# kekeliu-whu/Wildcat-SLAM

Measured on AMD Instinct MI355X. Metric: surfel-extract Mpts/s, higher is better.
Workload: dtype f64; 1 GPU; C2: 1M-pt single scan (G2 patch lattice, 999936 pts -> 31248 surfels) per GPU, voxel-grid + 3-level octree + per-cell 3x3 PCA; input = the reference's 48-byte hilti_ros::Point records, consumed in place; points_per_gpu=999936, surfels_per_gpu=31248, parallelism=sweep-per-gpu x1

## Files before the change

### wildcat-slam_amd/csrc/ctx.h

```cpp
#pragma once
#include <hip/hip_runtime.h>

#include <cstdarg>
#include <cstdio>
#include <cstdlib>
#include <cstring>
#include <string>
#include <vector>

#include "../../include/wildcat_hip.h"
#include "extract_plan.h"

struct wc_window_state;

struct wc_buf {
  void *p = nullptr;
  size_t cap = 0;
  bool pooled = false;
  bool plain = false;
};

#ifdef WC_DEV_KNOBS
#define WC_DBG(P, bit) ((P).dbg & (bit))
#else
#define WC_DBG(P, bit) 0
#endif

struct wc_dev_opts {
  int exact_sums = 0;
  int debug_skip = 0;
  int fx_merge_min = 3;
  int fx_split = -1;
  int no_bucket_sort = 0;
  int ex_sync = 0;
  int match_pair_serial = 0;
  int lm_dense = 0;
  int lm_side_stream = 1;
  int lm_one_collective = 0;
  int map_mom_pts = 1;
  int map_lin_groups = 0;
  int map_score_groups = 0;
  int map_cast_groups = 0;
  int map_carve_groups = 0;
  int map_remove_groups = 0;
  int map_absorb_groups = 0;
  int lm_dense_radius = 7;
  int lm_radius0 = -1;
};
inline bool wc_log_env(const char *name) { return getenv(name) != nullptr; }

struct wc_ctx {
  int device = 0;
  wc_params P;
  wc_dev_opts dev;
  bool pool_ok = false;
  hipMemPool_t pool = nullptr;
  hipStream_t own_stream = nullptr;
  hipStream_t stream = nullptr;
  hipEvent_t ev0 = nullptr, ev1 = nullptr;
  std::string err;
  wc_buf b_ex_ctrl;
  wc_buf b_keys[2], b_vals[2], b_sorttmp, b_slots, b_slot_ids, b_slot_keys[2], b_slot_idx[2], b_cand, b_cand_meta,
      b_status, b_misc[8], b_route[4], b_fx[10];
  double match_stats[8] = {0, 0, 0, 0, 0, 0, 0, 0};
  wc_buf b_kd[10];
  std::vector<wc_ctx *> batch_subs;
  wc_buf b_batch;
  wc_buf b_match_half;
  hipEvent_t ev_knn[2] = {nullptr, nullptr};
  wc_comm comm{};
  bool have_comm = false;
  void *rccl = nullptr;
  uint32_t *h_status_dev = nullptr;
  uint32_t *h_status = nullptr;
  unsigned long long mail_ticket = 0;
  wc_buf b_stage;
  void *h_stage = nullptr;
  size_t h_stage_cap = 0;
  double *h_mail = nullptr;
  ExSweep ex;
  ExMemory ex_mem;
  wc_window_state *win = nullptr;
  wc_ctx *aux = nullptr;
  hipEvent_t ev_aux = nullptr;
  hipEvent_t ev_pair = nullptr;
  void *pair_worker = nullptr;
  void (*pair_worker_free)(void *) = nullptr;
  void *pair_sync = nullptr;
  bool ex_prof = false;
  int ex_prof_mode = 0;
  hipEvent_t ex_ev[8] = {nullptr, nullptr, nullptr, nullptr, nullptr, nullptr, nullptr, nullptr};
};

struct wc_dev_guard {
  int prev = -1;
  bool switched = false;
  explicit wc_dev_guard(const wc_ctx *ctx) {
    if (ctx && hipGetDevice(&prev) == hipSuccess && prev != ctx->device) switched = hipSetDevice(ctx->device) == hipSuccess;
  }
  ~wc_dev_guard() {
    if (switched) (void)hipSetDevice(prev);
  }
  wc_dev_guard(const wc_dev_guard &) = delete;
  wc_dev_guard &operator=(const wc_dev_guard &) = delete;
};

inline int wc_fail(wc_ctx *ctx, int code, const char *fmt, ...) {
  char buf[512];
  va_list ap;
  va_start(ap, fmt);
  vsnprintf(buf, sizeof(buf), fmt, ap);
  va_end(ap);
  if (ctx) ctx->err = buf;
  return code;
}

#define WC_HIP(ctx, call)                                                                                   \
  do {                                                                                                      \
    hipError_t e_ = (call);                                                                                 \
    if (e_ != hipSuccess)                                                                                   \
      return wc_fail(ctx, WC_ERR_HIP, "%s failed: %s (%s:%d)", #call, hipGetErrorString(e_), __FILE__, __LINE__); \
  } while (0)

inline void wc_buf_release(wc_ctx *ctx, wc_buf &b) {
  if (!b.p) return;
  if (b.pooled && ctx && ctx->stream && hipFreeAsync(b.p, ctx->stream) == hipSuccess) {
  } else {
    if (ctx && ctx->stream) (void)hipStreamSynchronize(ctx->stream);
    (void)hipFree(b.p);
  }
  b.p = nullptr, b.cap = 0, b.pooled = false;
}
inline int wc_ensure(wc_ctx *ctx, wc_buf &b, size_t bytes) {
  if (bytes <= b.cap) return WC_OK;
  wc_buf_release(ctx, b);
  size_t want = bytes < ((size_t)64 << 20) ? 2 * bytes : bytes + bytes / 2;
  if (bytes >= ((size_t)64 << 10) && want < ((size_t)16 << 20)) want = (size_t)16 << 20;
  if (want < 4096) want = 4096;
  static const bool alloc_dbg = wc_log_env("WC_ALLOC_DEBUG");
  if (alloc_dbg) fprintf(stderr, "[alloc] %zu bytes wanted -> %zu\n", bytes, want);
  if (ctx->pool_ok && !b.plain && hipMallocFromPoolAsync(&b.p, want, ctx->pool, ctx->stream) == hipSuccess) {
    b.pooled = true;
  } else {
    (void)hipGetLastError();
    b.p = nullptr;
    WC_HIP(ctx, hipMalloc(&b.p, want));
    b.pooled = false;
  }
  b.cap = want;
  return WC_OK;
}
int wc_rccl_allreduce_on(wc_ctx *ctx, double *d_buf, uint64_t count, hipStream_t st);
#define WC_TRY(expr)            \
  do {                          \
    int rc_ = (expr);           \
    if (rc_ != WC_OK) return rc_; \
  } while (0)
```

### wildcat-slam_amd/csrc/ctx.hip

```cpp
#include "ctx.h"

#include <cmath>
#include <cstring>
#include <mutex>

extern "C" const char *wc_version(void) { return "wildcat_hip 0.1 (gfx950)"; }

extern "C" int wc_device_count(void) {
  int n = 0;
  if (hipGetDeviceCount(&n) != hipSuccess) return 0;
  return n;
}

extern "C" void wc_params_default(wc_params *p) {
  std::memset(p, 0, sizeof(*p));
  p->voxel_size = 0.8f;
  p->max_layer = 2;
  p->min_points = 20;
  p->planer_threshold = 0.01f;
  p->min_plane_likeness = 0.1;
  p->cluster_gap = 0.05;
  p->cluster_min_points = 20;
  p->center_scale = 1.0;
  p->angular_scale = 5.0 * M_PI / 180.0;
  p->surfel_dist_max = 0.1;
  p->knn_k = 10;
  p->time_diff_min = 0.06;
  p->surfel_sigma0 = 0.05 / 6;
  p->cauchy_a = 0.4;
  const double gn = 0.00015198973532354657, an = 0.006308226052016165;
  const double gw = 0.00011673723527962174, aw = 2.664506559330434e-06;
  const double rate = 200, k = 0.01;
  p->w_gyr = 1 / (gn * std::sqrt(rate)) * k;
  p->w_acc = 1 / (an * std::sqrt(rate)) * k;
  p->w_bg = 1 / (gw / std::sqrt(rate)) * k;
  p->w_ba = 1 / (aw / std::sqrt(rate)) * k;
  p->imu_dt = 1 / rate;
  p->max_iterations = 100;
  p->reference_quirks = 1;
  p->exact_sums = 0;
}

static int check_params(wc_ctx *ctx, const wc_params *p) {
  if (p->max_layer < 0 || p->max_layer > 2) return wc_fail(ctx, WC_ERR_ARG, "max_layer must be 0..2");
  if (!(p->voxel_size > 0)) return wc_fail(ctx, WC_ERR_ARG, "voxel_size must be positive");
  if (p->cluster_min_points < 1 || p->min_points < 0) return wc_fail(ctx, WC_ERR_ARG, "bad point thresholds");
  if (p->knn_k < 1 || p->knn_k > 16) return wc_fail(ctx, WC_ERR_ARG, "knn_k must be 1..16");
  return WC_OK;
}

namespace {
struct DevOpt {
  const char *name, *env;
  int wc_dev_opts::*field;
  bool flag_only;
};
const DevOpt kDevOpts[] = {
    {"exact_sums", "WC_EXACT_SUMS", &wc_dev_opts::exact_sums, true},
    {"debug_skip", "WC_DEBUG_SKIP", &wc_dev_opts::debug_skip, false},
    {"fx_merge_min", "WC_FX_MERGE_MIN", &wc_dev_opts::fx_merge_min, false},
    {"fx_split", "WC_FX_SPLIT", &wc_dev_opts::fx_split, false},
    {"no_bucket_sort", "WC_NO_BUCKET_SORT", &wc_dev_opts::no_bucket_sort, true},
    {"ex_sync", "WC_EX_SYNC", &wc_dev_opts::ex_sync, true},
    {"match_pair_serial", "WC_MATCH_PAIR_SERIAL", &wc_dev_opts::match_pair_serial, true},
    {"lm_dense", "WC_LM_DENSE", &wc_dev_opts::lm_dense, true},
    {"lm_one_collective", "WC_LM_ONE_COLLECTIVE", &wc_dev_opts::lm_one_collective, true},
    {"lm_side_stream", "WC_LM_SIDE_STREAM", &wc_dev_opts::lm_side_stream, false},
    {"map_mom_pts", "WC_MAP_MOM_PTS", &wc_dev_opts::map_mom_pts, false},
    {"map_lin_groups", "WC_MAP_LIN_GROUPS", &wc_dev_opts::map_lin_groups, false},
    {"map_score_groups", "WC_MAP_SCORE_GROUPS", &wc_dev_opts::map_score_groups, false},
    {"map_carve_groups", "WC_MAP_CARVE_GROUPS", &wc_dev_opts::map_carve_groups, false},
    {"map_cast_groups", "WC_MAP_CAST_GROUPS", &wc_dev_opts::map_cast_groups, false},
    {"map_absorb_groups", "WC_MAP_ABSORB_GROUPS", &wc_dev_opts::map_absorb_groups, false},
    {"map_remove_groups", "WC_MAP_REMOVE_GROUPS", &wc_dev_opts::map_remove_groups, false},
    {"lm_dense_radius", "WC_LM_DENSE_RADIUS", &wc_dev_opts::lm_dense_radius, false},
    {"lm_radius0", "WC_LM_RADIUS0", &wc_dev_opts::lm_radius0, false},
};
}

namespace {
struct DevPool {
  hipMemPool_t pool = nullptr;
  int refs = 0;
};
std::mutex g_pool_mu;
DevPool g_pools[64];
}
hipMemPool_t wc_pool_acquire(int device) {
  if (device < 0 || device >= 64) return nullptr;
  std::lock_guard<std::mutex> lk(g_pool_mu);
  DevPool &d = g_pools[device];
  if (!d.pool) {
    int supported = 0;
    if (hipDeviceGetAttribute(&supported, hipDeviceAttributeMemoryPoolsSupported, device) != hipSuccess || !supported) {
      (void)hipGetLastError();
      return nullptr;
    }
    hipMemPoolProps props;
    std::memset(&props, 0, sizeof(props));
    props.allocType = hipMemAllocationTypePinned;
    props.handleTypes = hipMemHandleTypeNone;
    props.location.type = hipMemLocationTypeDevice;
    props.location.id = device;
    hipMemPool_t p = nullptr;
    if (hipMemPoolCreate(&p, &props) != hipSuccess || !p) {
      (void)hipGetLastError();
      return nullptr;
    }
    uint64_t keep = ~0ull;
    if (hipMemPoolSetAttribute(p, hipMemPoolAttrReleaseThreshold, &keep) != hipSuccess) (void)hipGetLastError();
    d.pool = p;
  }
  ++d.refs;
  return d.pool;
}
void wc_pool_release(int device, hipMemPool_t pool) {
  if (!pool || device < 0 || device >= 64) return;
  std::lock_guard<std::mutex> lk(g_pool_mu);
  DevPool &d = g_pools[device];
  if (d.pool == pool && --d.refs == 0) {
    (void)hipMemPoolDestroy(d.pool);
    d.pool = nullptr;
  }
}

extern "C" int wc_ctx_create(const wc_params *params, int device, wc_ctx **out) {
  if (!out) return WC_ERR_ARG;
  *out = nullptr;
  int n = 0;
  if (hipGetDeviceCount(&n) != hipSuccess || n <= 0 || device < 0 || device >= n) return WC_ERR_NOGPU;
  wc_ctx *ctx = new wc_ctx;
  ctx->device = device;
  if (params)
    ctx->P = *params;
  else
    wc_params_default(&ctx->P);
  int rc = check_params(ctx, &ctx->P);
  if (rc != WC_OK) {
    delete ctx;
    return rc;
  }
  int prev_dev = -1;
  (void)hipGetDevice(&prev_dev);
  struct Restore {
    int d;
    ~Restore() {
      if (d >= 0) (void)hipSetDevice(d);
    }
  } restore{prev_dev};
  if (hipSetDevice(device) != hipSuccess || hipStreamCreateWithFlags(&ctx->own_stream, hipStreamNonBlocking) != hipSuccess ||
      hipEventCreate(&ctx->ev0) != hipSuccess || hipEventCreate(&ctx->ev1) != hipSuccess ||
      hipHostMalloc((void **)&ctx->h_status, 128 * sizeof(uint32_t)) != hipSuccess ||
      hipHostMalloc((void **)&ctx->h_mail, (64 + 4096) * sizeof(double)) != hipSuccess) {
    delete ctx;
    return WC_ERR_HIP;
  }
  ctx->stream = ctx->own_stream;
  {
    void *dp = nullptr;
    if (hipHostGetDevicePointer(&dp, ctx->h_status, 0) == hipSuccess) ctx->h_status_dev = (uint32_t *)dp;
    for (int q = 0; q < 128; ++q) ctx->h_status[q] = 0;
  }
  for (wc_buf &b : ctx->b_route) b.plain = true;
  ctx->b_status.plain = true;
  ctx->pool = wc_pool_acquire(device);
  ctx->pool_ok = ctx->pool != nullptr;
#ifdef WC_DEV_KNOBS
  for (const DevOpt &o : kDevOpts)
    if (const char *v = getenv(o.env)) ctx->dev.*(o.field) = o.flag_only ? 1 : atoi(v);
#endif
  *out = ctx;
  return WC_OK;
}

extern "C" int wc_ctx_set_dev_option(wc_ctx *ctx, const char *name, int value) {
  if (!ctx || !name) return wc_fail(ctx, WC_ERR_ARG, "%s: null or out-of-range argument", __func__);
  for (const DevOpt &o : kDevOpts)
    if (strcmp(o.name, name) == 0) {
      ctx->dev.*(o.field) = value;
      ex_reset_backoff(ctx->ex_mem);
      if (ctx->aux) ctx->aux->dev = ctx->dev;
      for (wc_ctx *sub : ctx->batch_subs) sub->dev = ctx->dev, ex_reset_backoff(sub->ex_mem);
      return WC_OK;
    }
  return wc_fail(ctx, WC_ERR_ARG, "wc_ctx_set_dev_option: unknown option '%s'", name);
}

void wc_window_free(wc_ctx *ctx);
extern "C" int wc_comm_rccl_destroy(wc_ctx *ctx);

extern "C" void wc_ctx_destroy(wc_ctx *ctx) {
  wc_dev_guard dg_(ctx);
  if (!ctx) return;
  (void)hipSetDevice(ctx->device);
  (void)hipStreamSynchronize(ctx->stream);
  if (ctx->pair_worker && ctx->pair_worker_free) ctx->pair_worker_free(ctx->pair_worker);
  ctx->pair_worker = nullptr;
  if (ctx->aux) {
    wc_ctx_destroy(ctx->aux);
    ctx->aux = nullptr;
  }
  if (ctx->ev_aux) (void)hipEventDestroy(ctx->ev_aux);
  if (ctx->ev_pair) (void)hipEventDestroy(ctx->ev_pair);
  for (hipEvent_t e : ctx->ev_knn)
    if (e) (void)hipEventDestroy(e);
  (void)wc_comm_rccl_destroy(ctx);
  wc_window_free(ctx);
  wc_buf *all[] = {&ctx->b_keys[0],      &ctx->b_keys[1],     &ctx->b_vals[0],     &ctx->b_vals[1],      &ctx->b_sorttmp,
                   &ctx->b_slots,        &ctx->b_slot_ids,    &ctx->b_slot_keys[0], &ctx->b_slot_keys[1], &ctx->b_slot_idx[0],
                   &ctx->b_slot_idx[1],  &ctx->b_cand,        &ctx->b_cand_meta,   &ctx->b_status,
                   &ctx->b_ex_ctrl};
  for (wc_buf *b : all) wc_buf_release(ctx, *b);
  for (wc_buf &b : ctx->b_misc) wc_buf_release(ctx, b);
  for (wc_buf &b : ctx->b_route) wc_buf_release(ctx, b);
  wc_buf_release(ctx, ctx->b_batch);
  for (wc_buf &b : ctx->b_kd) wc_buf_release(ctx, b);
  wc_buf_release(ctx, ctx->b_match_half);
  for (wc_ctx *sub : ctx->batch_subs) wc_ctx_destroy(sub);
  ctx->batch_subs.clear();
  for (wc_buf &b : ctx->b_fx) wc_buf_release(ctx, b);
  if (ctx->h_status) (void)hipHostFree(ctx->h_status);
  if (ctx->h_mail) (void)hipHostFree(ctx->h_mail);
  if (ctx->h_stage) (void)hipHostFree(ctx->h_stage);
  wc_buf_release(ctx, ctx->b_stage);
  (void)hipStreamSynchronize(ctx->stream);
  if (ctx->ev0) (void)hipEventDestroy(ctx->ev0);
  if (ctx->ev1) (void)hipEventDestroy(ctx->ev1);
  for (hipEvent_t e : ctx->ex_ev)
    if (e) (void)hipEventDestroy(e);
  if (ctx->own_stream) (void)hipStreamDestroy(ctx->own_stream);
  wc_pool_release(ctx->device, ctx->pool);
  delete ctx;
}

extern "C" const char *wc_last_error(const wc_ctx *ctx) { return ctx ? ctx->err.c_str() : "no context"; }

extern "C" int wc_ctx_set_stream(wc_ctx *ctx, void *hip_stream) {
  wc_dev_guard dg_(ctx);
  if (!ctx) return wc_fail(ctx, WC_ERR_ARG, "%s: null or out-of-range argument", __func__);
  WC_HIP(ctx, hipStreamSynchronize(ctx->stream));
  ctx->stream = hip_stream ? (hipStream_t)hip_stream : ctx->own_stream;
  return WC_OK;
}

extern "C" int wc_ctx_set_params(wc_ctx *ctx, const wc_params *params) {
  wc_dev_guard dg_(ctx);
  if (!ctx || !params) return wc_fail(ctx, WC_ERR_ARG, "%s: null or out-of-range argument", __func__);
  WC_TRY(check_params(ctx, params));
  ctx->P = *params;
  ex_reset_backoff(ctx->ex_mem);
  return WC_OK;
}

extern "C" int wc_dev_alloc(wc_ctx *ctx, size_t bytes, void **d_ptr) {
  wc_dev_guard dg_(ctx);
  if (!ctx || !d_ptr) return wc_fail(ctx, WC_ERR_ARG, "%s: null or out-of-range argument", __func__);
  WC_HIP(ctx, hipSetDevice(ctx->device));
  static const bool alloc_dbg = wc_log_env("WC_ALLOC_DEBUG");
  if (alloc_dbg) fprintf(stderr, "[alloc] wc_dev_alloc %zu bytes\n", bytes);
  WC_HIP(ctx, hipMalloc(d_ptr, bytes ? bytes : 1));
  return WC_OK;
}
extern "C" int wc_dev_free(wc_ctx *ctx, void *d_ptr) {
  wc_dev_guard dg_(ctx);
  if (!ctx) return wc_fail(ctx, WC_ERR_ARG, "%s: null or out-of-range argument", __func__);
  WC_HIP(ctx, hipStreamSynchronize(ctx->stream));
  WC_HIP(ctx, hipFree(d_ptr));
  return WC_OK;
}
extern "C" int wc_h2d(wc_ctx *ctx, void *d_dst, const void *h_src, size_t bytes) {
  wc_dev_guard dg_(ctx);
  if (!ctx) return wc_fail(ctx, WC_ERR_ARG, "%s: null or out-of-range argument", __func__);
  if (!bytes) return WC_OK;
  WC_HIP(ctx, hipMemcpyAsync(d_dst, h_src, bytes, hipMemcpyHostToDevice, ctx->stream));
  WC_HIP(ctx, hipStreamSynchronize(ctx->stream));
  return WC_OK;
}
extern "C" int wc_d2h(wc_ctx *ctx, void *h_dst, const void *d_src, size_t bytes) {
  wc_dev_guard dg_(ctx);
  if (!ctx) return wc_fail(ctx, WC_ERR_ARG, "%s: null or out-of-range argument", __func__);
  if (!bytes) return WC_OK;
  WC_HIP(ctx, hipMemcpyAsync(h_dst, d_src, bytes, hipMemcpyDeviceToHost, ctx->stream));
  WC_HIP(ctx, hipStreamSynchronize(ctx->stream));
  return WC_OK;
}
extern "C" int wc_d2d(wc_ctx *ctx, void *d_dst, const void *d_src, size_t bytes) {
  wc_dev_guard dg_(ctx);
  if (!ctx) return wc_fail(ctx, WC_ERR_ARG, "%s: null or out-of-range argument", __func__);
  if (!bytes) return WC_OK;
  WC_HIP(ctx, hipMemcpyAsync(d_dst, d_src, bytes, hipMemcpyDeviceToDevice, ctx->stream));
  WC_HIP(ctx, hipStreamSynchronize(ctx->stream));
  return WC_OK;
}
__global__ void __launch_bounds__(256) k_pack_strided(const uint32_t *src, uint32_t ew, uint32_t sw, uint64_t words, uint32_t *dst) {
  const uint64_t w = (uint64_t)blockIdx.x * blockDim.x + threadIdx.x;
  if (w < words) dst[w] = src[(w / ew) * sw + (w % ew)];
}
extern "C" int wc_d2h_strided(wc_ctx *ctx, void *h_dst, const void *d_src, size_t elem_bytes, size_t src_stride, size_t n) {
  wc_dev_guard dg_(ctx);
  if (!ctx || (n && (!h_dst || !d_src)) || elem_bytes == 0 || src_stride < elem_bytes)
    return wc_fail(ctx, WC_ERR_ARG, "%s: null or out-of-range argument", __func__);
  if (!n) return WC_OK;
  if (elem_bytes % 4 == 0 && src_stride % 4 == 0 && ((uintptr_t)d_src % 4) == 0 && n * elem_bytes <= ((size_t)64 << 20)) {
    const size_t bytes = n * elem_bytes;
    WC_TRY(wc_ensure(ctx, ctx->b_stage, bytes));
    if (ctx->h_stage_cap < bytes) {
      if (ctx->h_stage) (void)hipHostFree(ctx->h_stage);
      ctx->h_stage = nullptr, ctx->h_stage_cap = 0;
      const size_t want = std::max<size_t>(2 * bytes, (size_t)1 << 20);
      WC_HIP(ctx, hipHostMalloc(&ctx->h_stage, want));
      ctx->h_stage_cap = want;
    }
    const uint32_t ew = (uint32_t)(elem_bytes / 4), sw = (uint32_t)(src_stride / 4);
    const uint64_t words = (uint64_t)n * ew;
    k_pack_strided<<<(unsigned)((words + 255) / 256), 256, 0, ctx->stream>>>((const uint32_t *)d_src, ew, sw, words, (uint32_t *)ctx->b_stage.p);
    WC_HIP(ctx, hipGetLastError());
    WC_HIP(ctx, hipMemcpyAsync(ctx->h_stage, ctx->b_stage.p, bytes, hipMemcpyDeviceToHost, ctx->stream));
    WC_HIP(ctx, hipStreamSynchronize(ctx->stream));
    std::memcpy(h_dst, ctx->h_stage, bytes);
    return WC_OK;
  }
  WC_HIP(ctx, hipMemcpy2DAsync(h_dst, elem_bytes, d_src, src_stride, elem_bytes, n, hipMemcpyDeviceToHost, ctx->stream));
  WC_HIP(ctx, hipStreamSynchronize(ctx->stream));
  return WC_OK;
}
extern "C" int wc_memset(wc_ctx *ctx, void *d_dst, int value, size_t bytes) {
  wc_dev_guard dg_(ctx);
  if (!ctx) return wc_fail(ctx, WC_ERR_ARG, "%s: null or out-of-range argument", __func__);
  if (!bytes) return WC_OK;
  WC_HIP(ctx, hipMemsetAsync(d_dst, value, bytes, ctx->stream));
  return WC_OK;
}
extern "C" int wc_sync(wc_ctx *ctx) {
  wc_dev_guard dg_(ctx);
  if (!ctx) return wc_fail(ctx, WC_ERR_ARG, "%s: null or out-of-range argument", __func__);
  WC_HIP(ctx, hipStreamSynchronize(ctx->stream));
  return WC_OK;
}
extern "C" int wc_timer_start(wc_ctx *ctx) {
  wc_dev_guard dg_(ctx);
  if (!ctx) return wc_fail(ctx, WC_ERR_ARG, "%s: null or out-of-range argument", __func__);
  WC_HIP(ctx, hipEventRecord(ctx->ev0, ctx->stream));
  return WC_OK;
}
extern "C" int wc_timer_stop_ms(wc_ctx *ctx, float *h_ms) {
  wc_dev_guard dg_(ctx);
  if (!ctx || !h_ms) return wc_fail(ctx, WC_ERR_ARG, "%s: null or out-of-range argument", __func__);
  WC_HIP(ctx, hipEventRecord(ctx->ev1, ctx->stream));
  WC_HIP(ctx, hipEventSynchronize(ctx->ev1));
  WC_HIP(ctx, hipEventElapsedTime(h_ms, ctx->ev0, ctx->ev1));
  return WC_OK;
}

int wc_touch_extract();
int wc_touch_match();
int wc_touch_poses();
int wc_touch_sweep();
int wc_touch_route();
int wc_touch_window();
int wc_match_pair_prepare(wc_ctx *ctx);

extern "C" int wc_ctx_warmup(wc_ctx *ctx, size_t reserve_bytes) {
  wc_dev_guard dg_(ctx);
  if (!ctx) return wc_fail(ctx, WC_ERR_ARG, "%s: null or out-of-range argument", __func__);
// ... 35 lines not shown
```

### wildcat-slam_amd/csrc/extract.hip

```cpp
#include <hip/hip_runtime.h>
#include <type_traits>

#include <chrono>
#include <cstdlib>
#include <cstring>
#include <rocprim/rocprim.hpp>

#include "ctx.h"
#include "dmath.h"

namespace {

constexpr int kMom = 11;
constexpr int kProdStride = 66;
constexpr unsigned kRootsGrid = 256 * 16;
constexpr unsigned kEmitGrid = 256 * 8;
constexpr unsigned kRoots2Grid = 256 * 4;
constexpr int kTile = 2048;

struct ExParams {
  double vs;
  float vs_f;
  int max_layer;
  int min_points;
// ... 1479 lines not shown
    if (lane == 0) atomicAdd(&status[5], runs_part);
  }
  if (nb > bin_cap || nb > lds_cap) {
    if (lane == 0) raise_flag(status, nb > bin_cap ? kFlagBucketOverflow : kFlagLdsOverflow);
    nb = 0;
  }
  if (nb <= 64) {
    if ((uint32_t)lane < nb) s_a[lane] = first;
    __builtin_amdgcn_wave_barrier();
    if ((uint32_t)lane < nb) {
      uint32_t rank = 0;
      for (uint32_t j = 0; j < nb; ++j) rank += (s_a[j] < first) ? 1u : 0u;
      s_b[rank] = first;
    }
  } else {
    uint32_t N = 128;
    while (N < nb) N <<= 1;
    s_b[lane] = first;
    for (uint32_t i = lane + 64; i < N; i += 64) s_b[i] = (i < nb) ? bin[i] : ~0ull;
    __builtin_amdgcn_wave_barrier();
    for (uint32_t k = 2; k <= N; k <<= 1)
      for (uint32_t j = k >> 1; j > 0; j >>= 1) {
        for (uint32_t p = lane; p < N / 2; p += 64) {
          const uint32_t i = 2 * p - (p & (j - 1)), l = i + j;
          const uint64_t x = s_b[i], y = s_b[l];
          if ((x > y) == ((i & k) == 0)) {
            s_b[i] = y;
            s_b[l] = x;
          }
        }
        __builtin_amdgcn_wave_barrier();
      }
  }
  __builtin_amdgcn_wave_barrier();
  uint32_t carry = 0;
  for (uint32_t i0 = 0; i0 < nb; i0 += 64) {
    const uint32_t i = i0 + lane;
    const uint64_t c = (i < nb) ? s_b[i] : 0ull;
    const uint32_t l = (i < nb) ? comp_len(c) : 0u;
    uint32_t inc = l;
    for (int off = 1; off < 64; off <<= 1) {
      const uint32_t v = __shfl_up(inc, off);
      if (lane >= off) inc += v;
    }
    if (i < nb) {
      s_off[i] = carry + inc - l;
      bin[i] = c;
      run_off[(size_t)b * bin_cap + i] = carry + inc - l;
    }
    carry += __shfl(inc, 63);
  }
  __builtin_amdgcn_wave_barrier();
  uint32_t *s_list = (uint32_t *)s_a;
  uint32_t nlive = 0, next_head = nb;
  for (int i0 = (int)((nb + 63) / 64) * 64 - 64; i0 >= 0; i0 -= 64) {
    const uint32_t r = (uint32_t)i0 + lane;
    const bool in = r < nb;
    const uint32_t rest = in ? comp_rest(s_b[r]) : 0u;
    const bool head = in && (r == 0 || comp_rest(s_b[r - 1]) != rest);
    const unsigned long long hm = __ballot(head);
    const unsigned long long above = (lane == 63) ? 0ull : (hm >> (lane + 1));
    const uint32_t r2 = above ? r + (uint32_t)__ffsll((long long)above) : next_head;
    const uint32_t seg = (r2 < nb ? s_off[min(r2, nb - 1)] : total) - (in ? s_off[r] : 0u);
    const bool live = head && seg > (uint32_t)min_points;
    const unsigned long long lm = __ballot(live);
    if (live) s_list[nlive + (uint32_t)__popcll(lm & ((1ull << lane) - 1ull))] = r | (r2 << 16);
    nlive += (uint32_t)__popcll(lm);
    if (hm) next_head = (uint32_t)i0 + (uint32_t)__ffsll((long long)hm) - 1u;
  }
  if (lane == 0) s_live[w] = nlive;
  __syncthreads();
  const uint32_t pbase0 = s_red[0] + s_red[1] + s_red[2] + s_red[3];
  const uint32_t pbase = pbase0 + before;
  const uint32_t first_slot = pbase0 / (uint32_t)(min_points + 1);
  uint32_t lbase = 0;
  for (int j = 0; j < w; ++j) lbase += s_live[j];
  if (t == 0) {
    root_cnt[blockIdx.x] = s_live[0] + s_live[1] + s_live[2] + s_live[3];
    root_first[blockIdx.x] = first_slot;
  }
  for (uint32_t k = lane; k < nlive; k += 64) {
    const uint32_t r = s_list[k] & 0xFFFFu, r2 = s_list[k] >> 16;
    const uint32_t seg = (r2 < nb ? s_off[r2] : total) - s_off[r];
    head_slots[first_slot + lbase + k] = HeadRec{pbase + s_off[r], b * bin_cap + r, r2 - r, seg};
  }
}

inline uint32_t pt_bin_cap(uint64_t n) {
  uint32_t cap = 64;
  while (cap < kPtBinMax && (uint64_t)cap * kBuckets < 32 * n) cap *= 2;
  return cap;
}

constexpr uint32_t kCtrlStatus = 0, kCtrlCounts = 64, kCtrlRoots = kCtrlCounts + 2 * kBuckets, kCtrlBins = kCtrlRoots + 2 * (kBuckets / 4),
                   kCtrlFx = kCtrlBins + kBuckets, kCtrlWords = kCtrlFx + 4 * 16 * 32;

int clear_ctrl(wc_ctx *ctx) {
  WC_TRY(wc_ensure(ctx, ctx->b_ex_ctrl, kCtrlWords * 4));
  uint32_t *ctrl = (uint32_t *)ctx->b_ex_ctrl.p;
  InitArgs I{};
  void *dp = nullptr;
  if (hipHostGetDevicePointer(&dp, ctx->h_status, 0) != hipSuccess) dp = nullptr;
  const unsigned long long a = (unsigned long long)dp;
  I.p[0] = ctrl, I.nw[0] = 8, I.val[0] = 0u;
  I.p[1] = ctrl + 10, I.nw[1] = kCtrlRoots - 10, I.val[1] = 0u;
  I.p[2] = ctrl + 8, I.nw[2] = 1, I.val[2] = (uint32_t)a;
  I.p[3] = ctrl + 9, I.nw[3] = 1, I.val[3] = (uint32_t)(a >> 32);
  I.p[4] = ctrl + kCtrlBins, I.nw[4] = kBuckets + 4 * 16 * 32, I.val[4] = 0u;
  k_init<<<(kCtrlRoots + 255) / 256, 256, 0, ctx->stream>>>(I);
  WC_HIP(ctx, hipGetLastError());
  return WC_OK;
}

int point_sort_runs(wc_ctx *ctx, const wc_points &pts, double vs, HeadRec *head_slots, int min_points, uint32_t *status) {
  hipStream_t st = ctx->stream;
  const uint64_t n = pts.n;
  const uint32_t cap = pt_bin_cap(n);
  const uint32_t lds_cap = std::min(cap, std::max(64u, ctx->ex_mem.lds_cap));
  WC_TRY(wc_ensure(ctx, ctx->b_misc[1], (uint64_t)kBuckets * cap * 8));
  WC_TRY(wc_ensure(ctx, ctx->b_misc[3], (uint64_t)kBuckets * cap * 4));
  uint32_t *counts = (uint32_t *)ctx->b_ex_ctrl.p + kCtrlCounts;
  const unsigned tiles = (unsigned)((n + kTile - 1) / kTile);
  const size_t lds = (size_t)4 * lds_cap * 20;
  if (!ctx->ex_mem.bucket_attr_set) {
    WC_HIP(ctx, hipFuncSetAttribute((const void *)k_pt_bucket, hipFuncAttributeMaxDynamicSharedMemorySize, (int)(4 * kPtBinMax * 20)));
    ctx->ex_mem.bucket_attr_set = true;
  }
  k_pt_runs<<<tiles, kRunThreads, 0, st>>>(pts, vs, n, counts, (uint64_t *)ctx->b_misc[1].p, cap, status);
  k_pt_bucket<<<kBuckets / 4, 256, lds, st>>>((uint64_t *)ctx->b_misc[1].p, cap, lds_cap, counts, (uint32_t *)ctx->b_misc[3].p, head_slots,
                                             counts + 2 * kBuckets, counts + 2 * kBuckets + kBuckets / 4, min_points, status);
  WC_HIP(ctx, hipGetLastError());
  return WC_OK;
}

template <typename K>
int sort_pairs(wc_ctx *ctx, K *kin, K *kout, uint32_t *vin, uint32_t *vout, size_t n, unsigned end_bit) {
  using cfg = rocprim::radix_sort_config<rocprim::default_config, rocprim::default_config, rocprim::default_config, 0>;
  size_t tmp = 0;
  WC_HIP(ctx, rocprim::radix_sort_pairs<cfg>(nullptr, tmp, kin, kout, vin, vout, n, 0u, end_bit, ctx->stream));
  WC_TRY(wc_ensure(ctx, ctx->b_sorttmp, tmp));
  tmp = ctx->b_sorttmp.cap;
  WC_HIP(ctx, rocprim::radix_sort_pairs<cfg>(ctx->b_sorttmp.p, tmp, kin, kout, vin, vout, n, 0u, end_bit, ctx->stream));
  return WC_OK;
}

#include "extract_fast.inc"
#include "extract_split.inc"

int fx_ensure_zero(wc_ctx *ctx, wc_buf &b, size_t bytes) {
  if (bytes <= b.cap) return WC_OK;
  WC_TRY(wc_ensure(ctx, b, bytes));
  WC_HIP(ctx, hipMemsetAsync(b.p, 0, b.cap, ctx->stream));
  return WC_OK;
}

bool fx_applicable(const wc_ctx *ctx, uint64_t n, double t_lo, double t_hi) {
  const wc_params &P = ctx->P;
  if (P.exact_sums || ctx->dev.exact_sums) return false;
  if (n < 64 || !(P.voxel_size > 0.0f) || P.voxel_size >= 0.99f) return false;
  if (!(P.cluster_gap > 1e-6) || !(t_hi > t_lo)) return false;
  if ((t_hi - t_lo) / (P.cluster_gap * 0.999) >= 1048000.0) return false;
  return true;
}

ExParams ex_params(const wc_ctx *ctx) {
  const wc_params &P = ctx->P;
  ExParams E{};
  E.vs = (double)P.voxel_size, E.vs_f = P.voxel_size, E.max_layer = P.max_layer, E.min_points = P.min_points;
  E.thr = (double)P.planer_threshold, E.min_like = P.min_plane_likeness;
  for (int i = 0; i < 3; ++i) E.view[i] = P.view_point[i];
  E.gap = P.cluster_gap, E.cluster_min = P.cluster_min_points;
  E.t_lo_bits = ordered_bits_host(ctx->ex.t_lo);
  E.t_span_bits = ordered_bits_host(ctx->ex.t_hi) - E.t_lo_bits;
  E.dbg = ctx->dev.debug_skip;
  E.merge_min = ctx->dev.fx_merge_min;
  return E;
}

void ex_mark(wc_ctx *ctx, int i) {
  if (ctx->ex_prof && (ctx->ex_prof_mode != 2 || i == 1 || i == 5)) (void)hipEventRecord(ctx->ex_ev[i], ctx->stream);
}

template <typename Args>
void ex_keep_for_tail(wc_ctx *ctx, const Args &A, int (*tail)(wc_ctx *, bool)) {
  static_assert(sizeof(Args) <= sizeof(ctx->ex.roots_args), "extract_plan.h: roots_args too small");
  std::memcpy(ctx->ex.roots_args, &A, sizeof(A));
  ctx->ex.tail = tail;
}

int fx_tail(wc_ctx *ctx, bool layer2);

int run_pipeline_fast(wc_ctx *ctx) {
  const wc_params &P = ctx->P;
  ExMemory &M = ctx->ex_mem;
  const wc_points &pts = ctx->ex.pts;
  const double t_lo = ctx->ex.t_lo, t_hi = ctx->ex.t_hi;
  const uint64_t n = pts.n;
  hipStream_t st = ctx->stream;
  FxArgs A;
  std::memset(&A, 0, sizeof(A));
  A.P = ex_params(ctx);
  A.pts = pts;
  A.t_lo = t_lo;
  int e = 0;
  (void)std::frexp(t_hi - t_lo, &e);
  A.tick = std::ldexp(1.0, 40 - e), A.inv_tick = std::ldexp(1.0, e - 40);
  A.inv_w = 1.0 / (P.cluster_gap * 0.999);
  A.inv_span = 1.0 / (t_hi - t_lo);
  A.inv_vs = 1.0 / (double)P.voxel_size;
  A.qs = 4294967296.0, A.inv_q = 1.0 / 4294967296.0, A.inv_qq = std::ldexp(1.0, -44);
  {
    const double vs = (double)P.voxel_size;
    A.band0 = 1e-14 + 3.0 * (std::ldexp(1.0, -45) + 2.0 * std::ldexp(1.0, -33) * vs + 16.0 * std::ldexp(1.0, -53) * (0.5 * vs) * (0.5 * vs));
  }
  uint32_t mr = 1024;
  while ((uint64_t)mr * 8 < n) mr *= 2;
  A.mr_per = mr / kFxSub, A.mq_per = std::max(64u, mr / 2 / kFxSub);
  uint32_t tr = 2048;
  while ((uint64_t)tr * 4 < n) tr *= 2;
  A.tr_mask = tr - 1;
  A.static_map = n <= 2000000ull ? 1u : 0u;
  {
    const uintptr_t px = (uintptr_t)pts.xyz, pt = (uintptr_t)pts.time;
    if (pts.xyz_stride == 48u && pts.time_stride == 48u && pt == px + 24u && px % 16u == 0u)
      A.fmt = 1u;
    else if (pts.xyz_stride == 12u && pts.time_stride == 8u && px % 16u == 0u && pt % 16u == 0u)
      A.fmt = 2u;
  }
  const unsigned tiles = ex_fx_tiles(n);
  A.rec_tiles = tiles;
  const uint64_t spill_full = ((uint64_t)tiles + 7) / 8 * kFxTile;
  A.spill_per = (uint32_t)((n <= 8000000ull || M.fx_spill_full) ? spill_full : std::max<uint64_t>(1024, n / 32));
  A.rec_cap = tiles * (uint32_t)kFxRecTile + 8u * A.spill_per;
  const uint64_t total_slots = ex_total_slots(n, P.max_layer, P.cluster_min_points, (uint64_t)kFxSub * 256);
  const uint32_t bin_cap = ex_slot_bin_cap(total_slots);
  WC_TRY(fx_ensure_zero(ctx, ctx->b_fx[0], (size_t)tr * 4));
  WC_TRY(wc_ensure(ctx, ctx->b_fx[1], (size_t)mr * 4));
  WC_TRY(fx_ensure_zero(ctx, ctx->b_fx[2], (size_t)tr * kFxBlockW * 8));
  WC_TRY(fx_ensure_zero(ctx, ctx->b_fx[3], (size_t)A.mq_per * kFxSub * kFxBlockW * 8));
  WC_TRY(wc_ensure(ctx, ctx->b_fx[4], (size_t)2 * A.rec_cap * kFxRecW * 8));
  const unsigned ngrid = ex_fx_node_grid(n);
  WC_TRY(wc_ensure(ctx, ctx->b_fx[6], (size_t)ngrid * kFxJobCap * kFxJobW * 8));
  ctx->ex.fx_split = ctx->ex.batch_defer || (ctx->dev.fx_split >= 0 ? ctx->dev.fx_split != 0 : !A.static_map);
  if (ctx->ex.fx_split) {
    A.static_map = 0u;
    A.jobpool_per = (uint32_t)std::max<uint64_t>(4096, n / (uint64_t)std::max(1, P.cluster_min_points) / 2);
    WC_TRY(wc_ensure(ctx, ctx->b_fx[7], ((size_t)mr / 8 + 2) * kFxNodeW * 64 * 8));
    WC_TRY(wc_ensure(ctx, ctx->b_fx[8], ((size_t)mr / 8 + 2) * kFxDescW * 4));
    WC_TRY(wc_ensure(ctx, ctx->b_fx[9], (size_t)8 * A.jobpool_per * kFxJobW * 8));
    A.nodes = (unsigned long long *)ctx->b_fx[7].p, A.wdesc = (uint32_t *)ctx->b_fx[8].p, A.jobpool = (unsigned long long *)ctx->b_fx[9].p;
  }
  WC_TRY(wc_ensure(ctx, ctx->b_slots, total_slots * sizeof(wc_surfel)));
  WC_TRY(wc_ensure(ctx, ctx->b_slot_ids, total_slots * sizeof(wc_surfel_id)));
  WC_TRY(wc_ensure(ctx, ctx->b_slot_keys[1], (uint64_t)kBuckets * bin_cap * 8));
  if (M.fx_dirty) {
    for (int i : {0, 2, 3}) WC_HIP(ctx, hipMemsetAsync(ctx->b_fx[i].p, 0, ctx->b_fx[i].cap, st));
    M.fx_dirty = false;
  }
  WC_TRY(wc_ensure(ctx, ctx->b_fx[5], (size_t)2 * kCtrlWords * 4));
  if (!M.fx_ctrl_ready) {
    WC_HIP(ctx, hipMemsetAsync(ctx->b_fx[5].p, 0, (size_t)2 * kCtrlWords * 4, st));
    const unsigned long long a = (unsigned long long)ctx->h_status_dev;
    const uint32_t addr[2] = {(uint32_t)a, (uint32_t)(a >> 32)};
    for (int b = 0; b < 2; ++b)
      WC_HIP(ctx, hipMemcpyAsync((uint32_t *)ctx->b_fx[5].p + (size_t)b * kCtrlWords + 8, addr, 8, hipMemcpyHostToDevice, st));
    WC_HIP(ctx, hipStreamSynchronize(st));
    M.fx_ctrl_ready = true;
    M.fx_parity = 0;
  }
  uint32_t *ctrl = (uint32_t *)ctx->b_fx[5].p + (size_t)M.fx_parity * kCtrlWords;
  for (int q = 0; q < 64; ++q) ctx->h_status[q] = 0;
  A.rkey = (uint32_t *)ctx->b_fx[0].p, A.rlist = (uint32_t *)ctx->b_fx[1].p;
  A.blk = (unsigned long long *)ctx->b_fx[2].p, A.blk2 = (unsigned long long *)ctx->b_fx[3].p;
  A.rec = (unsigned long long *)ctx->b_fx[4].p;
  A.jobs = (unsigned long long *)ctx->b_fx[6].p;
  A.status = ctrl + kCtrlStatus;
  A.cnt = ctrl + kCtrlFx;
  A.slots = (wc_surfel *)ctx->b_slots.p, A.slot_ids = (wc_surfel_id *)ctx->b_slot_ids.p;
  A.slots_per = (uint32_t)std::min<uint64_t>(total_slots / kFxSub, 0x7FFFFFFFu);
  A.slot_counts = ctrl + kCtrlBins;
  A.slot_bins = (uint64_t *)ctx->b_slot_keys[1].p;
  A.slot_bin_cap = bin_cap;
  ex_mark(ctx, 0);
  ex_mark(ctx, 1);
  static const bool dbg = wc_log_env("WC_FX_DEBUG");
  auto dbg_sync = [&](const char *what) {
    if (!dbg) return;
    fprintf(stderr, "[fx] %s ...", what);
    const hipError_t e = hipStreamSynchronize(st);
    uint32_t w[64], c[4 * 16 * 32];
    (void)hipMemcpy(w, A.status, sizeof(w), hipMemcpyDeviceToHost);
    (void)hipMemcpy(c, A.cnt, sizeof(c), hipMemcpyDeviceToHost);
    uint32_t r = 0, q = 0, sl = 0, sp = 0;
    for (int j = 0; j < 16; ++j) r += c[j * 32], q += c[(16 + j) * 32], sl += c[(32 + j) * 32], sp += c[(48 + j) * 32];
    fprintf(stderr, " %s flags=%u roots=%u nodes2=%u slots=%u spill=%u\n", hipGetErrorString(e), w[1], r, q, sl, sp);
  };
  if (dbg) fprintf(stderr, "[fx] n=%llu tiles=%u mr_per=%u mq_per=%u tr=%u slots_per=%u bin_cap=%u\n", (unsigned long long)n, tiles, A.mr_per, A.mq_per, tr, A.slots_per, bin_cap);
  ex_keep_for_tail(ctx, A, &fx_tail);
  if (ctx->ex.batch_defer) {
    ctx->ex.layer2_done = P.max_layer >= 2 && M.last_splits > 0;
    ctx->ex.deferred = true;
    return WC_OK;
  }
  k_fx_acc<1><<<tiles, kFxThreads, 0, st>>>(A);
  dbg_sync("k_fx_acc<1>");
  ex_mark(ctx, 2);
  if (M.fx_long_lists) k_fx_merge<1><<<std::min<unsigned>(ngrid * 2u, 8192u), 128, 0, st>>>(A);
  if (ctx->ex.fx_split) {
    k_fx_walk<1><<<ngrid, 64, 0, st>>>(A);
    dbg_sync("k_fx_walk<1>");
    k_fx_test<1><<<ngrid, 64, 0, st>>>(A);
  } else {
    k_fx_nodes<1><<<ngrid, 64, 0, st>>>(A);
  }
  dbg_sync("k_fx_nodes<1>");
  ex_mark(ctx, 3);
  return fx_tail(ctx, P.max_layer >= 2 && M.last_splits > 0);
}

constexpr int kMailTicket = 120;
__global__ void k_ex_ticket(uint32_t *host_word, uint32_t ticket) {
  __hip_atomic_store(host_word, ticket, __ATOMIC_RELEASE, __HIP_MEMORY_SCOPE_SYSTEM);
}

int fx_tail(wc_ctx *ctx, bool layer2) {
  hipStream_t st = ctx->stream;
  FxArgs A;
  std::memcpy(&A, ctx->ex.roots_args, sizeof(A));
  ExMemory &M = ctx->ex_mem;
  if (layer2) {
    k_fx_acc<2><<<ex_fx_tiles(A.pts.n), kFxThreads, 0, st>>>(A);
    if (M.fx_long_lists2) k_fx_merge<2><<<std::min(8192u, std::max(64u, M.last_splits)), 128, 0, st>>>(A);
    const unsigned g2 = ex_fx_layer2_grid(ex_fx_node_grid(A.pts.n), M.last_splits);
    if (ctx->ex.fx_split) {
      k_fx_walk<2><<<g2, 64, 0, st>>>(A);
      k_fx_test<2><<<g2, 64, 0, st>>>(A);
    } else {
      k_fx_nodes<2><<<g2, 64, 0, st>>>(A);
    }
  }
  ctx->ex.layer2_done = layer2;
  ex_mark(ctx, 4);
  uint32_t *next_ctrl = (uint32_t *)ctx->b_fx[5].p + (size_t)(M.fx_parity ^ 1) * kCtrlWords;
  static_assert(kCtrlWords <= (kBuckets / 4) * 256, "k_slot_emit's grid covers the control block");
  k_slot_emit<<<kBuckets / 4, 256, 0, st>>>(A.slot_counts, A.slot_bins, A.slot_bin_cap, (const wc_surfel *)ctx->b_slots.p,
                                           (const wc_surfel_id *)ctx->b_slot_ids.p, A.status, ctx->ex.d_out, ctx->ex.d_ids, ctx->ex.cap, next_ctrl,
                                           kCtrlWords);
  ex_mark(ctx, 5);
  ctx->ex.ticket = 0;
  if (ctx->h_status_dev && !ctx->ex_prof && !ctx->dev.ex_sync) {
    if (++M.ticket_seq == 0u) ++M.ticket_seq;
    ctx->ex.ticket = M.ticket_seq;
    k_ex_ticket<<<1, 1, 0, st>>>(ctx->h_status_dev + kMailTicket, ctx->ex.ticket);
  }
  static const bool fx_dbg = wc_log_env("WC_FX_DEBUG");
  if (fx_dbg) fprintf(stderr, "[fx] k_slot_emit (layer2=%d) ... %s\n", (int)layer2, hipGetErrorString(hipStreamSynchronize(st)));
  WC_HIP(ctx, hipGetLastError());
  return WC_OK;
}

template <typename K, bool RUNS>
int pipeline_tail(wc_ctx *ctx, bool layer2) {
  hipStream_t st = ctx->stream;
  RootsArgs A;
  memcpy(&A, ctx->ex.roots_args, sizeof(A));
  uint32_t *status = A.status;
  const uint64_t cap = ctx->ex.cap, total_slots = A.total_slots;
  const bool fast_slots = A.slot_counts != nullptr;
  if (layer2) {
    const unsigned grid2 = std::min(kRoots2Grid, std::max(64u, ctx->ex_mem.last_splits));
    if constexpr (RUNS) {
      if (ctx->ex_mem.unordered)
        k_roots_banks<K, 2, true><<<grid2, 64, 0, st>>>(A, (const K *)ctx->b_keys[1].p);
      else
        k_roots<K, 2><<<grid2, 64, 0, st>>>(A);
    } else {
      k_roots_banks<K, 2, false><<<grid2, 64, 0, st>>>(A, (const K *)ctx->b_keys[1].p);
    }
  }
  ctx->ex.layer2_done = layer2;
  ex_mark(ctx, 4);
  if (fast_slots) {
    k_slot_emit<<<kBuckets / 4, 256, 0, st>>>(A.slot_counts, A.slot_bins, A.slot_bin_cap, (const wc_surfel *)ctx->b_slots.p,
                                             (const wc_surfel_id *)ctx->b_slot_ids.p, status, ctx->ex.d_out, ctx->ex.d_ids, cap, nullptr, 0u);
  } else {
    k_iota<<<(unsigned)((total_slots + 255) / 256), 256, 0, st>>>((uint32_t *)ctx->b_slot_idx[0].p, total_slots);
    WC_TRY(sort_pairs<uint64_t>(ctx, (uint64_t *)ctx->b_slot_keys[0].p, (uint64_t *)ctx->b_slot_keys[1].p,
                                (uint32_t *)ctx->b_slot_idx[0].p, (uint32_t *)ctx->b_slot_idx[1].p, total_slots,
                                ctx->ex.slot_end_bit));
    k_fix_ties<<<(unsigned)((total_slots + 255) / 256), 256, 0, st>>>((const uint64_t *)ctx->b_slot_keys[1].p, (uint32_t *)ctx->b_slot_idx[1].p,
                                                                     total_slots, (const wc_surfel_id *)ctx->b_slot_ids.p);
    const uint64_t gth = std::min<uint64_t>(total_slots, cap) * 10;
    if (gth)
      k_gather<<<(unsigned)((gth + 255) / 256), 256, 0, st>>>((const uint32_t *)ctx->b_slot_idx[1].p, (const wc_surfel *)ctx->b_slots.p,
                                                             (const wc_surfel_id *)ctx->b_slot_ids.p, status, ctx->ex.d_out, ctx->ex.d_ids, cap);
  }
  ex_mark(ctx, 5);
  if (!fast_slots) WC_HIP(ctx, hipMemcpyAsync(ctx->h_status, status, 32, hipMemcpyDeviceToHost, st));
  WC_HIP(ctx, hipGetLastError());
  return WC_OK;
}

template <typename K>
int run_pipeline(wc_ctx *ctx, const ExPath &path) {
  const wc_params &P = ctx->P;
  const wc_points &pts = ctx->ex.pts;
  const uint64_t n = pts.n;
  hipStream_t st = ctx->stream;
  const ExParams E = ex_params(ctx);
  unsigned tbits = 1;
  while (tbits < 64 && (E.t_span_bits >> tbits)) ++tbits;
  const unsigned slot_end_bit = tbits >= 63 ? 64 : tbits + 1;

  const uint64_t total_slots = ex_total_slots(n, P.max_layer, P.cluster_min_points, 0);
  WC_TRY(wc_ensure(ctx, ctx->b_keys[0], n * sizeof(K)));
  WC_TRY(wc_ensure(ctx, ctx->b_keys[1], n * sizeof(K)));
  WC_TRY(wc_ensure(ctx, ctx->b_vals[0], n * 4));
  WC_TRY(wc_ensure(ctx, ctx->b_vals[1], n * 4));
  WC_TRY(wc_ensure(ctx, ctx->b_cand, total_slots * kMom * 8));
  WC_TRY(wc_ensure(ctx, ctx->b_cand_meta, total_slots * 4));
  WC_TRY(wc_ensure(ctx, ctx->b_slots, total_slots * sizeof(wc_surfel)));
  WC_TRY(wc_ensure(ctx, ctx->b_slot_ids, total_slots * sizeof(wc_surfel_id)));
  WC_TRY(wc_ensure(ctx, ctx->b_slot_keys[0], total_slots * 8));
  WC_TRY(wc_ensure(ctx, ctx->b_slot_keys[1], total_slots * 8));
  WC_TRY(wc_ensure(ctx, ctx->b_slot_idx[0], total_slots * 4));
  WC_TRY(wc_ensure(ctx, ctx->b_slot_idx[1], total_slots * 4));
  WC_TRY(wc_ensure(ctx, ctx->b_misc[0], (n / (uint64_t)(P.min_points + 1) + 2) * sizeof(HeadRec)));
  const bool precleared = ctx->ex_mem.precleared && ctx->b_ex_ctrl.p;
  ctx->ex_mem.precleared = false;
  if (!precleared) WC_TRY(clear_ctrl(ctx));
  for (int q = 0; q < 16; ++q) ctx->h_status[q] = 0;
  uint32_t *status = (uint32_t *)ctx->b_ex_ctrl.p + kCtrlStatus;

  ex_mark(ctx, 0);
  const bool fast_slots = path.bin_order && tbits <= 31 && total_slots < (1ull << 31);
  const uint32_t bin_cap = ex_slot_bin_cap(total_slots);
  const unsigned g256 = (unsigned)((n + 255) / 256);
  const bool fast_pts = path.run_sort && sizeof(K) == 4;
  if (fast_pts || fast_slots) {
    WC_TRY(wc_ensure(ctx, ctx->b_slot_keys[1], (uint64_t)kBuckets * bin_cap * 8));
  }
  const uint32_t nslots = (uint32_t)(n / (uint64_t)(P.min_points + 1) + 1);
  if (!fast_slots || !fast_pts) {
    InitArgs I{};
    int r = 0;
    auto fill = [&](void *p, uint64_t words, uint32_t v) { I.p[r] = (uint32_t *)p, I.nw[r] = (uint32_t)words, I.val[r] = v, ++r; };
    if (!fast_slots) fill(ctx->b_slot_keys[0].p, total_slots * 2, 0xFFFFFFFFu);
    if (!fast_pts) fill(ctx->b_misc[0].p, (uint64_t)nslots * 4, 0xFFFFFFFFu);
    uint32_t mx = 0;
    for (int q = 0; q < r; ++q) mx = std::max(mx, I.nw[q]);
    k_init<<<(mx + 255) / 256, 256, 0, st>>>(I);
  }
  ex_mark(ctx, 1);
  if (fast_pts) {
    WC_TRY(point_sort_runs(ctx, pts, E.vs, (HeadRec *)ctx->b_misc[0].p, P.min_points, status));
  } else {
    k_keygen<K><<<g256, 256, 0, st>>>(pts, E.vs, (K *)ctx->b_keys[0].p, (uint32_t *)ctx->b_vals[0].p, status);
    WC_TRY(sort_pairs<K>(ctx, (K *)ctx->b_keys[0].p, (K *)ctx->b_keys[1].p, (uint32_t *)ctx->b_vals[0].p,
                         (uint32_t *)ctx->b_vals[1].p, n, 3 * KeyTraits<K>::bits + 1));
  }
  RootsArgs A;
  A.pts = pts;
  A.P = E;
  A.n = n;
  A.vals = (const uint32_t *)ctx->b_vals[1].p;
  A.cand = (double *)ctx->b_cand.p;
  A.cand_meta = (uint32_t *)ctx->b_cand_meta.p;
  A.slots = (wc_surfel *)ctx->b_slots.p;
  A.slot_ids = (wc_surfel_id *)ctx->b_slot_ids.p;
  A.slot_keys = (uint64_t *)ctx->b_slot_keys[0].p;
  A.total_slots = total_slots;
  A.status = status;
  A.slot_counts = fast_slots ? (uint32_t *)ctx->b_ex_ctrl.p + kCtrlBins : nullptr;
  A.slot_shift = tbits > 12 ? tbits - 12 : 0u;
  A.slot_bins = (uint64_t *)ctx->b_slot_keys[1].p;
  A.runs = (const uint64_t *)ctx->b_misc[1].p;
  A.run_off = (const uint32_t *)ctx->b_misc[3].p;
  A.run_cap = pt_bin_cap(n);
  A.root_cnt = (const uint32_t *)ctx->b_ex_ctrl.p + kCtrlRoots;
  A.root_first = A.root_cnt + kBuckets / 4;
  A.slot_bin_cap = bin_cap;
  A.heads = (const HeadRec *)ctx->b_misc[0].p;
  A.nslots = nslots;
  if (!fast_pts) k_heads<K><<<g256, 256, 0, st>>>((const K *)ctx->b_keys[1].p, n, P.min_points, (HeadRec *)ctx->b_misc[0].p);
  ex_mark(ctx, 2);
  WC_TRY(wc_ensure(ctx, ctx->b_misc[5], (size_t)A.nslots * sizeof(SplitJob)));
  A.split_jobs = (SplitJob *)ctx->b_misc[5].p;
  A.prof = nullptr;
#ifdef WC_PROF_ROOTS
  WC_TRY(wc_ensure(ctx, ctx->b_misc[6], (size_t)A.nslots * 32));
  WC_HIP(ctx, hipMemsetAsync(ctx->b_misc[6].p, 0, (size_t)A.nslots * 32, st));
  A.prof = (uint32_t *)ctx->b_misc[6].p;
#endif
  WC_TRY(wc_ensure(ctx, ctx->b_misc[7], (size_t)A.nslots * (9 * kMom * 8 + 4)));
  A.node_tot = (double *)ctx->b_misc[7].p;
  A.root_ncand = (uint32_t *)(A.node_tot + (size_t)A.nslots * 9 * kMom);
  const K *skeys = (const K *)ctx->b_keys[1].p;
  if (fast_pts) {
    if constexpr (sizeof(K) == 4) {
      if (ctx->ex_mem.unordered)
        k_roots_banks<K, 1, true><<<kRootsGrid, 64, 0, st>>>(A, skeys);
      else
        k_roots<K, 1><<<kRootsGrid, 64, 0, st>>>(A);
      ex_mark(ctx, 3);
      k_roots_emit<K, true><<<kEmitGrid, 64, 0, st>>>(A, skeys);
    }
  } else {
    k_roots_banks<K, 1, false><<<kRootsGrid, 64, 0, st>>>(A, skeys);
    ex_mark(ctx, 3);
    k_roots_emit<K, false><<<kEmitGrid, 64, 0, st>>>(A, skeys);
  }
  ex_keep_for_tail(ctx, A, fast_pts ? &pipeline_tail<K, (sizeof(K) == 4)> : &pipeline_tail<K, false>);
  ctx->ex.slot_end_bit = slot_end_bit;
  return ctx->ex.tail(ctx, ctx->ex_mem.last_splits > 0);
}

int enqueue_path(wc_ctx *ctx, const ExPath &path) {
  ctx->ex.path = path;
  ++ctx->ex.runs;
  const int rc = path.fx ? run_pipeline_fast(ctx) : path.wide ? run_pipeline<uint64_t>(ctx, path) : run_pipeline<uint32_t>(ctx, path);
  if (path.fx && rc != WC_OK) ctx->ex_mem.fx_dirty = true;
  return rc;
}

int ex_wait(wc_ctx *ctx) {
  bool arrived = false;
  if (const uint32_t ticket = ctx->ex.ticket) {
    ctx->ex.ticket = 0;
    const uint32_t *w = (const uint32_t *)ctx->h_status + kMailTicket;
    const auto t0 = std::chrono::steady_clock::now();
    for (uint32_t spin = 0; !arrived; ++spin) {
      arrived = __atomic_load_n(w, __ATOMIC_ACQUIRE) == ticket;
      if ((spin & 1023u) == 1023u && std::chrono::steady_clock::now() - t0 > std::chrono::milliseconds(20)) break;
    }
  }
  if (!arrived) WC_HIP(ctx, hipStreamSynchronize(ctx->stream));
  for (int i = 0; i < 7; ++i)
    if (ctx->h_status[8 + i]) ctx->h_status[1] |= 1u << i;
  return WC_OK;
}

}

extern "C" int wc_voxel_keys(wc_ctx *ctx, const wc_points *pts, int32_t *d_keys_xyz) {
  wc_dev_guard dg_(ctx);
  if (!ctx || !pts || !d_keys_xyz) return wc_fail(ctx, WC_ERR_ARG, "%s: null or out-of-range argument", __func__);
  if (pts->n == 0) return WC_OK;
  k_voxel_keys<<<(unsigned)((pts->n + 255) / 256), 256, 0, ctx->stream>>>(*pts, (double)ctx->P.voxel_size, d_keys_xyz);
  WC_HIP(ctx, hipGetLastError());
  WC_HIP(ctx, hipStreamSynchronize(ctx->stream));
  return WC_OK;
}

extern "C" int wc_extract_surfels_enqueue(wc_ctx *ctx, const wc_points *pts, double t_lo, double t_hi, wc_surfel *d_out,
                                          wc_surfel_id *d_ids, uint64_t cap) {
  wc_dev_guard dg_(ctx);
  if (!ctx || !pts) return wc_fail(ctx, WC_ERR_ARG, "%s: null or out-of-range argument", __func__);
  if (pts->n >= (1ull << 32)) return wc_fail(ctx, WC_ERR_ARG, "at most 2^32-1 points per call");
  ctx->ex.active = true;
  ctx->ex.ticket = 0;
  ctx->ex.pts = *pts;
  ctx->ex.d_out = d_out, ctx->ex.d_ids = d_ids, ctx->ex.cap = cap;
  ctx->ex.path = ExPath{}, ctx->ex.runs = 0;
  for (int q = 0; q < 16; ++q) ctx->h_status[q] = 0;
  if (pts->n == 0) return WC_OK;
  if (t_lo > t_hi) {
    WC_HIP(ctx, hipMemcpyAsync(&ctx->h_mail[0], pts->time, 8, hipMemcpyDeviceToHost, ctx->stream));
    WC_HIP(ctx, hipMemcpyAsync(&ctx->h_mail[1], (const char *)pts->time + (pts->n - 1) * pts->time_stride, 8,
                               hipMemcpyDeviceToHost, ctx->stream));
    WC_HIP(ctx, hipStreamSynchronize(ctx->stream));
    t_lo = ctx->h_mail[0];
    t_hi = ctx->h_mail[1];
  }
  {
    const double mag = std::max(std::fabs(t_lo), std::fabs(t_hi));
    const double m = 4096.0 * (std::nextafter(mag, INFINITY) - mag);
    t_lo -= m;
    t_hi += m;
  }
  ctx->ex.t_lo = t_lo, ctx->ex.t_hi = t_hi;
  return enqueue_path(ctx, ex_first_path(ctx->ex_mem, fx_applicable(ctx, pts->n, t_lo, t_hi), ctx->dev.no_bucket_sort != 0));
}

extern "C" int wc_extract_surfels_finish(wc_ctx *ctx, uint64_t *h_n_out) {
  wc_dev_guard dg_(ctx);
  if (!ctx || !ctx->ex.active) return wc_fail(ctx, WC_ERR_ARG, "%s: null or out-of-range argument", __func__);
  ExSweep &S = ctx->ex;
  ExMemory &M = ctx->ex_mem;
  S.active = false;
  if (h_n_out) *h_n_out = 0;
  if (S.pts.n == 0) return WC_OK;
  WC_TRY(ex_wait(ctx));
  if (S.path.fx) {
    if (!S.layer2_done && ctx->P.max_layer >= 2 && ctx->h_status[4] > 0 && !(ctx->h_status[1] & (kFlagFxFallback | kFlagKeyRange))) {
      M.last_splits = ctx->h_status[4];
      WC_TRY(fx_tail(ctx, true));
      WC_TRY(ex_wait(ctx));
    }
    M.last_splits = ctx->h_status[4];
  }
  ExPath path = S.path;
  while (ex_next_path(path, ctx->h_status[1], ctx->h_status + 32, M)) {
    WC_TRY(enqueue_path(ctx, path));
    WC_TRY(ex_wait(ctx));
  }
  if (path.fx) {
    M.fx_long_lists = ctx->h_status[15] != 0u;
    M.fx_long_lists2 = ctx->h_status[16] != 0u;
    M.fx_parity ^= 1;
  } else {
    if (!S.layer2_done && ctx->h_status[4] > 0 && S.tail) {
      M.last_splits = ctx->h_status[4];
      WC_TRY(S.tail(ctx, true));
      WC_TRY(ex_wait(ctx));
    }
    M.last_splits = ctx->h_status[4];
    ex_learn_unordered(M, path, ctx->h_status[5], S.pts.n);
    if (clear_ctrl(ctx) == WC_OK) M.precleared = true;
  }
  const uint32_t flags = ctx->h_status[1], n_out = ctx->h_status[0];
  if (h_n_out) *h_n_out = n_out;
  if (flags & kFlagKeyRange) return wc_fail(ctx, WC_ERR_ARG, "point cloud extent exceeds 2^20 root voxels");
  if (flags & kFlagSlotOverflow) return wc_fail(ctx, WC_ERR_HIP, "internal: candidate slot overflow");
  if (flags & kFlagTimeRange) return wc_fail(ctx, WC_ERR_ARG, "surfel timestamp outside the [t_lo, t_hi] hint");
  if (n_out > S.cap) return wc_fail(ctx, WC_ERR_CAPACITY, "output capacity %llu < %u surfels", (unsigned long long)S.cap, n_out);
  return WC_OK;
}

extern "C" int wc_extract_surfels(wc_ctx *ctx, const wc_points *pts, double t_lo, double t_hi, wc_surfel *d_out,
                                  wc_surfel_id *d_ids, uint64_t cap, uint64_t *h_n_out) {
  wc_dev_guard dg_(ctx);
  WC_TRY(wc_extract_surfels_enqueue(ctx, pts, t_lo, t_hi, d_out, d_ids, cap));
  return wc_extract_surfels_finish(ctx, h_n_out);
}

extern "C" int wc_extract_surfels_batch_enqueue(wc_ctx *ctx, const wc_sweep_job *jobs, int K) {
  wc_dev_guard dg_(ctx);
  if (!ctx || !jobs || K < 1 || K > 64) return wc_fail(ctx, WC_ERR_ARG, "%s: null or out-of-range argument", __func__);
  while ((int)ctx->batch_subs.size() < K) {
    wc_ctx *sub = nullptr;
    const int rc = wc_ctx_create(&ctx->P, ctx->device, &sub);
    if (rc != WC_OK) return wc_fail(ctx, rc, "wc_extract_surfels_batch: no sub-context");
    ctx->batch_subs.push_back(sub);
  }
  hipStream_t st = ctx->stream;
  const size_t o_emit = (sizeof(FxArgs) * K + 15) & ~(size_t)15, o_tab = (o_emit + sizeof(SlotEmitArgs) * K + 15) & ~(size_t)15;
  const size_t bytes = o_tab + (size_t)(3 * (K + 1) + K) * 4;
  std::vector<unsigned char> host(bytes, 0);
  FxArgs *args = (FxArgs *)host.data();
  SlotEmitArgs *emit = (SlotEmitArgs *)(host.data() + o_emit);
  uint32_t *s_acc = (uint32_t *)(host.data() + o_tab), *s_nodes = s_acc + (K + 1), *s_g2 = s_nodes + (K + 1), *flags = s_g2 + (K + 1);
  int Kd = 0;
  bool any_l2 = false, any_merge = false;
  for (int k = 0; k < K; ++k) {
    wc_ctx *sub = ctx->batch_subs[k];
    if (sub->stream != st) WC_TRY(wc_ctx_set_stream(sub, st));
    if (std::memcmp(&sub->P, &ctx->P, sizeof(wc_params)) != 0) WC_TRY(wc_ctx_set_params(sub, &ctx->P));
    if (std::memcmp(&sub->dev, &ctx->dev, sizeof(wc_dev_opts)) != 0) {
      sub->dev = ctx->dev;
      ex_reset_backoff(sub->ex_mem);
    }
    sub->ex.batch_defer = true;
    sub->ex.deferred = false;
    const int rc = wc_extract_surfels_enqueue(sub, &jobs[k].pts, jobs[k].t_lo, jobs[k].t_hi, jobs[k].d_out, jobs[k].d_ids, jobs[k].cap);
    sub->ex.batch_defer = false;
    if (rc != WC_OK) {
      for (int j = 0; j <= k; ++j) {
        wc_ctx *pj = ctx->batch_subs[j];
        if (pj->ex.deferred || j == k) pj->ex_mem.fx_dirty = true, pj->ex.active = false, pj->ex.deferred = false;
      }
      return wc_fail(ctx, rc, "wc_extract_surfels_batch (sweep %d): %s", k, wc_last_error(sub));
    }
    if (!sub->ex.deferred) continue;
    FxArgs &A = args[Kd];
    std::memcpy(&A, sub->ex.roots_args, sizeof(A));
    const unsigned ngrid = ex_fx_batch_node_grid(A.pts.n);
    s_acc[Kd + 1] = s_acc[Kd] + ex_fx_tiles(A.pts.n);
    s_nodes[Kd + 1] = s_nodes[Kd] + ngrid;
    s_g2[Kd + 1] = s_g2[Kd] + ex_fx_layer2_grid(ngrid, sub->ex_mem.last_splits);
    const uint32_t f = (sub->ex.layer2_done ? 1u : 0u) | ((sub->ex_mem.fx_long_lists || sub->ex_mem.fx_long_lists2) ? 2u : 0u);
    flags[Kd] = f;
    any_l2 = any_l2 || (f & 1u);
    any_merge = any_merge || (f & 2u);
    uint32_t *next_ctrl = (uint32_t *)sub->b_fx[5].p + (size_t)(sub->ex_mem.fx_parity ^ 1) * kCtrlWords;
    emit[Kd++] = SlotEmitArgs{A.slot_counts, A.slot_bins, A.slot_bin_cap, (const wc_surfel *)sub->b_slots.p, (const wc_surfel_id *)sub->b_slot_ids.p,
                              A.status, sub->ex.d_out, sub->ex.d_ids, sub->ex.cap, next_ctrl, (uint32_t)kCtrlWords};
  }
  if (Kd == 0) return WC_OK;
  WC_TRY(wc_ensure(ctx, ctx->b_batch, bytes));
  WC_HIP(ctx, hipMemcpyAsync(ctx->b_batch.p, host.data(), bytes, hipMemcpyHostToDevice, st));
  WC_HIP(ctx, hipStreamSynchronize(st));
  const unsigned char *d = (const unsigned char *)ctx->b_batch.p;
  const uint32_t *dt = (const uint32_t *)(d + o_tab);
  FxBatch B;
  B.args = (const FxArgs *)d, B.K = Kd, B.flags = dt + 3 * (K + 1);
  B.start = dt;
  k_fx_acc_b<1><<<s_acc[Kd], kFxThreads, 0, st>>>(B);
  B.start = dt + (K + 1);
  if (any_merge) k_fx_merge_b<1><<<s_nodes[Kd], 128, 0, st>>>(B);
  k_fx_walk_b<1><<<s_nodes[Kd], 64, 0, st>>>(B);
  k_fx_test_b<1><<<s_nodes[Kd], 64, 0, st>>>(B);
  if (any_l2) {
    B.start = dt;
    k_fx_acc_b<2><<<s_acc[Kd], kFxThreads, 0, st>>>(B);
    B.start = dt + 2 * (K + 1);
    if (any_merge) k_fx_merge_b<2><<<s_g2[Kd], 128, 0, st>>>(B);
    k_fx_walk_b<2><<<s_g2[Kd], 64, 0, st>>>(B);
    k_fx_test_b<2><<<s_g2[Kd], 64, 0, st>>>(B);
  }
  k_slot_emit_b<<<(unsigned)Kd * (kBuckets / 4), 256, 0, st>>>((const SlotEmitArgs *)(d + o_emit), Kd);
  WC_HIP(ctx, hipGetLastError());
  return WC_OK;
}

extern "C" int wc_extract_surfels_batch_finish(wc_ctx *ctx, uint64_t *h_n_out, int K) {
  wc_dev_guard dg_(ctx);
  if (!ctx || !h_n_out || K < 1 || K > (int)ctx->batch_subs.size()) return wc_fail(ctx, WC_ERR_ARG, "%s: null or out-of-range argument", __func__);
  int first_rc = WC_OK;
  for (int k = 0; k < K; ++k) {
    wc_ctx *sub = ctx->batch_subs[k];
    h_n_out[k] = 0;
    if (!sub->ex.active) continue;
    const int rc = wc_extract_surfels_finish(sub, &h_n_out[k]);
    if (rc != WC_OK && first_rc == WC_OK) first_rc = wc_fail(ctx, rc, "wc_extract_surfels_batch (sweep %d): %s", k, wc_last_error(sub));
  }
  return first_rc;
}

extern "C" int wc_extract_profile(wc_ctx *ctx, int enable) {
  wc_dev_guard dg_(ctx);
  if (!ctx) return wc_fail(ctx, WC_ERR_ARG, "%s: null or out-of-range argument", __func__);
  if (enable && !ctx->ex_ev[0])
    for (int i = 0; i < 8; ++i) WC_HIP(ctx, hipEventCreate(&ctx->ex_ev[i]));
  ctx->ex_prof = enable != 0;
  ctx->ex_prof_mode = enable;
  return WC_OK;
}

extern "C" int wc_extract_stage_ms(wc_ctx *ctx, float *h_ms5) {
  wc_dev_guard dg_(ctx);
  if (!ctx || !h_ms5 || !ctx->ex_ev[0]) return wc_fail(ctx, WC_ERR_ARG, "%s: null or out-of-range argument", __func__);
  WC_HIP(ctx, hipEventSynchronize(ctx->ex_ev[5]));
  if (ctx->ex_prof_mode == 2) {
    for (int i = 0; i < 5; ++i) h_ms5[i] = 0.f;
    WC_HIP(ctx, hipEventElapsedTime(&h_ms5[1], ctx->ex_ev[1], ctx->ex_ev[5]));
    return WC_OK;
  }
  for (int i = 0; i < 5; ++i) WC_HIP(ctx, hipEventElapsedTime(&h_ms5[i], ctx->ex_ev[i], ctx->ex_ev[i + 1]));
  return WC_OK;
}

extern "C" int wc_debug_status(wc_ctx *ctx, uint32_t *h_out64) {
  wc_dev_guard dg_(ctx);
  if (!ctx || !h_out64) return wc_fail(ctx, WC_ERR_ARG, "%s: null or out-of-range argument", __func__);
  for (int i = 0; i < 64; ++i) h_out64[i] = i < 16 ? ctx->h_status[i] : 0u;
  h_out64[56] = ctx->ex.runs;
  h_out64[57] = ex_path_bits(ctx->ex.path);
  h_out64[58] = ctx->ex_mem.lds_cap;
  h_out64[59] = ctx->ex_mem.fx_long_lists ? 1u : 0u;
  h_out64[60] = ctx->ex_mem.fx_fallbacks;
  h_out64[61] = ctx->ex.path.fx ? 1u : 0u;
  h_out64[62] = ctx->ex_mem.fx_last_flags;
  h_out64[63] = ctx->ex_mem.fx_last_why;
#ifdef WC_PROF_ROOTS
  const size_t nslots = ctx->ex.pts.n / (size_t)(ctx->P.min_points + 1) + 1;
  std::vector<uint32_t> rows(nslots * 8);
  WC_HIP(ctx, hipMemcpy(rows.data(), ctx->b_misc[6].p, nslots * 32, hipMemcpyDeviceToHost));
  double sum[8] = {0};
  uint32_t cnt = 0;
  for (size_t r = 0; r < nslots; ++r)
    if (rows[r * 8 + 1]) {
      ++cnt;
      for (int i = 0; i < 8; ++i) sum[i] += rows[r * 8 + i];
    }
  for (int i = 0; i < 8; ++i) h_out64[16 + i] = cnt ? (uint32_t)(sum[i] / cnt) : 0;
  h_out64[24] = cnt;
#endif
  return WC_OK;
}

namespace {
struct FxEigOut {
  double ev[3];
  double vec[3];
  double accepted;
  double spare;
};
__global__ void k_selftest_fx_eig3(const double *a9, FxEigOut *o) {
  wc::M3 a, v;
  for (int i = 0; i < 3; ++i)
    for (int j = 0; j < 3; ++j) a.m[i][j] = a9[3 * i + j];
  bool acc = false;
  fx_eig3(a, o->ev, v, &acc);
  for (int i = 0; i < 3; ++i) o->vec[i] = v.m[i][0];
  o->accepted = acc ? 1.0 : 0.0;
  o->spare = 0.0;
}
}

extern "C" int wc_selftest_fx_eig3(wc_ctx *ctx, const double a9[9], double out8[8]) {
  if (!ctx || !a9 || !out8) return wc_fail(ctx, WC_ERR_ARG, "%s: null argument", __func__);
  wc_dev_guard dg_(ctx);
  WC_TRY(wc_ensure(ctx, ctx->b_status, 1024));
  double *d_in = (double *)ctx->b_status.p;
  FxEigOut *d_out = (FxEigOut *)((char *)ctx->b_status.p + 128);
  FxEigOut o;
  WC_HIP(ctx, hipMemcpyAsync(d_in, a9, 9 * 8, hipMemcpyHostToDevice, ctx->stream));
  k_selftest_fx_eig3<<<1, 1, 0, ctx->stream>>>(d_in, d_out);
  WC_HIP(ctx, hipGetLastError());
  WC_HIP(ctx, hipMemcpyAsync(&o, d_out, sizeof(o), hipMemcpyDeviceToHost, ctx->stream));
  WC_HIP(ctx, hipStreamSynchronize(ctx->stream));
  std::memcpy(out8, &o, sizeof(o));
  return WC_OK;
}

int wc_touch_extract() {
  hipFuncAttributes a;
  return hipFuncGetAttributes(&a, (const void *)k_voxel_keys) == hipSuccess ? WC_OK : WC_ERR_HIP;
}
```

### wildcat-slam_amd/csrc/extract_fast.inc

```

constexpr int kFxLds = 256;
constexpr int kFxLdsProbe = 12;
constexpr int kFxDirect = 16;
constexpr int kFxRecTile = kFxLds + (kFxThreads / 64) * 4 * kFxDirect;
constexpr int kFxSlots = 16;
constexpr int kFxRecW = 16;
constexpr int kFxHdrW = 16;
constexpr int kFxBlockW = kFxHdrW + 8 * kFxSlots / 2;
constexpr uint32_t kFxStRoots = 0, kFxStNodes2 = 1, kFxStSlots = 2, kFxStSpillBank = 3;
constexpr int kFxCntStride = 32;
constexpr int kFxCntWords = 4 * kFxSub * kFxCntStride;
constexpr unsigned long long kFxTMax = 0xFFFFFFFFFFFFull;
constexpr double kFxMagic = 6755399441055744.0, kFxMagic2 = 7083549724304467820544.0;
constexpr unsigned long long kFxMagicBits = 0x4338000000000000ull;
constexpr uint32_t kFxMagicHi = 0x43380000u, kFxMagic2Hi = 0x44780000u;

struct FxArgs {
  wc_points pts;
  ExParams P;
  double t_lo;
  double tick, inv_tick;
  double inv_w;
  double inv_span;
  double inv_vs;
  double qs, inv_q, inv_qq;
  double band0;
  uint32_t *rkey;
  uint32_t *rlist;
  uint32_t tr_mask;
  uint32_t static_map;
  unsigned long long *blk;
  unsigned long long *blk2;
  unsigned long long *rec;
  uint32_t rec_tiles;
  uint32_t spill_per;
  uint32_t rec_cap;
  uint32_t mr_per, mq_per;
  uint32_t fmt;
  uint32_t *status;
  uint32_t *cnt;
  unsigned long long *jobs;
  unsigned long long *nodes;
  uint32_t *wdesc;
  unsigned long long *jobpool;
  uint32_t jobpool_per;
  wc_surfel *slots;
  wc_surfel_id *slot_ids;
  uint32_t slots_per;
  uint32_t *slot_counts;
  uint64_t *slot_bins;
  uint32_t slot_bin_cap;
};

__device__ __forceinline__ void fx_fallback(uint32_t *status, int why) {
  raise_flag(status, kFlagFxFallback);
  uint32_t *hm = host_mailbox(status);
  if (hm) hm[32 + why] = 1u;
}
__device__ __forceinline__ uint32_t *fx_cnt(const FxArgs &A, uint32_t bank, uint32_t j) { return A.cnt + (bank * kFxSub + j) * kFxCntStride; }

__device__ __forceinline__ uint32_t fx_hash32(uint32_t k) {
  k ^= k >> 16;
  k *= 0x7FEB352Du;
  k ^= k >> 15;
  k *= 0x846CA68Bu;
  k ^= k >> 16;
  return k;
}

__device__ __forceinline__ int fx_vox(double p, double vs, double inv_vs) {
  const double q = p * inv_vs;
  const double r = rint(q);
  if (fabs(q - r) > 1e-9 * (fabs(r) + 1.0)) return (int)floor(q);
  return (int)floor(p / vs);
}

constexpr int kFxStMaxProbe = 20;
__device__ __forceinline__ uint32_t fx_root_slot(const FxArgs &A, uint32_t key1, uint32_t sub, bool insert, uint32_t maxprobe = 0u) {
  uint32_t slot = fx_hash32(key1) & A.tr_mask;
  for (int probe = 0; probe < 64; ++probe) {
    uint32_t k;
    if (insert) {
      k = atomicCAS(&A.rkey[slot], 0u, key1);
      if (k == 0u) {
        if (probe) atomicMax(&A.status[kFxStMaxProbe], (uint32_t)probe);
        const uint32_t local = atomicAdd(fx_cnt(A, kFxStRoots, sub), 1u);
        if (local < A.mr_per)
          A.rlist[sub * A.mr_per + local] = slot;
        else
          fx_fallback(A.status, 0);
        return slot;
      }
    } else {
      k = __hip_atomic_load(&A.rkey[slot], __ATOMIC_RELAXED, __HIP_MEMORY_SCOPE_AGENT);
      if (k == 0u && (uint32_t)probe >= maxprobe) return 0xFFFFFFFFu;
    }
    if (k == key1) return slot;
    slot = (slot + 1u) & A.tr_mask;
  }
  fx_fallback(A.status, 1);
  return 0xFFFFFFFFu;
}

struct FxPart {
  uint32_t n;
  long long st, s[3], ss[6];
  unsigned long long tmin_inv, tmax_p1;
};
__device__ __forceinline__ void fx_zero(FxPart &a) {
  a.n = 0, a.st = 0, a.tmin_inv = 0, a.tmax_p1 = 0;
  for (int i = 0; i < 3; ++i) a.s[i] = 0;
  for (int i = 0; i < 6; ++i) a.ss[i] = 0;
}
__device__ __forceinline__ void fx_acc(FxPart &a, const FxPart &b) {
  a.n += b.n, a.st += b.st;
  for (int i = 0; i < 3; ++i) a.s[i] += b.s[i];
  for (int i = 0; i < 6; ++i) a.ss[i] += b.ss[i];
  a.tmin_inv = max(a.tmin_inv, b.tmin_inv);
  a.tmax_p1 = max(a.tmax_p1, b.tmax_p1);
}

__device__ __forceinline__ void fx_add_cell(unsigned long long *cell, const FxPart &a) {
  atomicAdd((uint32_t *)cell, a.n);
  atomicAdd(&cell[1], (unsigned long long)a.st);
  for (int i = 0; i < 3; ++i) atomicAdd(&cell[2 + i], (unsigned long long)a.s[i]);
  for (int i = 0; i < 6; ++i) atomicAdd(&cell[5 + i], (unsigned long long)a.ss[i]);
  atomicMax(&cell[11], a.tmin_inv);
  atomicMax(&cell[12], a.tmax_p1);
}

struct FxEarly {
  uint32_t key1, s0, found;
  int lead;
};
template <int LEVEL>
__device__ __forceinline__ void fx_push(const FxArgs &A, bool active, unsigned long long code, const FxPart &a, uint32_t sub, uint32_t ridx,
                                        const FxEarly &E) {
  const int lane = threadIdx.x & 63;
  unsigned long long *blk = nullptr;
  uint32_t oct, bin, pkey;
  if (LEVEL == 1) {
    pkey = (uint32_t)(code & 0x3FFFFFFFull) + 1u;
    oct = (uint32_t)(code >> 30) & 7u;
    bin = (uint32_t)(code >> 33) & 0xFFFFFu;
  } else {
    pkey = (uint32_t)(code & 0xFFFFFFFull) + 1u;
    oct = (uint32_t)(code >> 28) & 7u;
    bin = (uint32_t)(code >> 31) & 0xFFFFFu;
  }
  int lead = lane;
  uint32_t gmb = bin;
  {
    unsigned long long todo = __ballot(active);
    while (todo) {
      const int first = __ffsll((long long)todo) - 1;
      const uint32_t k0 = (uint32_t)__shfl((int)pkey, first);
      const bool mine = active && pkey == k0;
      uint32_t mb = mine ? bin : 0xFFFFFFFFu;
      for (int m = 1; m < 64; m <<= 1) mb = min(mb, (uint32_t)__shfl_xor((int)mb, m));
      if (mine) lead = first, gmb = mb;
      todo &= ~__ballot(mine);
    }
  }
  const bool leader = active && lane == lead;
  uint32_t slot = 0xFFFFFFFFu;
  bool created = false;
  const uint32_t e_found = (uint32_t)__shfl((int)E.found, E.lead);
  const bool e_have = LEVEL == 1 && E.key1 != 0u && E.key1 == pkey;
  if (leader) {
    if (LEVEL == 1) {
      if (WC_DBG(A.P, 64)) {
        slot = fx_hash32(pkey) & A.tr_mask;
      } else {
        uint32_t s = fx_hash32(pkey) & A.tr_mask;
        int probe = 0;
        if (e_have) {
          if (e_found == 0u || e_found == pkey) {
            slot = s;
          } else {
            s = (s + 1u) & A.tr_mask;
            probe = 1;
          }
        }
        for (; slot == 0xFFFFFFFFu && probe < 64; ++probe) {
          const uint32_t k = atomicCAS(&A.rkey[s], 0u, pkey);
          if (k == 0u || k == pkey) {
            slot = s;
            created = k == 0u;
            if (created && probe) atomicMax(&A.status[kFxStMaxProbe], (uint32_t)probe);
            break;
          }
          s = (s + 1u) & A.tr_mask;
        }
        if (slot == 0xFFFFFFFFu) fx_fallback(A.status, 2);
      }
    } else {
      slot = pkey - 1u;
    }
  }
  const unsigned long long cm = __ballot(created);
  uint32_t list_base = 0;
  const int cfirst = cm ? __ffsll((long long)cm) - 1 : 0;
  if (cm && lane == cfirst) list_base = atomicAdd(fx_cnt(A, kFxStRoots, sub), (uint32_t)__popcll(cm));
  if (leader && slot != 0xFFFFFFFFu && !(WC_DBG(A.P, 8))) {
    unsigned long long *b0 = (LEVEL == 1 ? A.blk : A.blk2) + (size_t)slot * kFxBlockW;
    atomicMax((uint32_t *)b0 + 2, 0xFFFFFFFFu - gmb);
  }
  const uint32_t myslot = (uint32_t)__shfl((int)slot, lead);
  uint32_t old = 0;
  const bool ok = active && myslot != 0xFFFFFFFFu;
  if (ok) {
    blk = (LEVEL == 1 ? A.blk : A.blk2) + (size_t)myslot * kFxBlockW;
    uint32_t *heads = (uint32_t *)(blk + kFxHdrW);
    if (!(WC_DBG(A.P, 32))) old = atomicExch(&heads[oct * kFxSlots + (bin & (kFxSlots - 1))], ridx + 1u);
  }
  if (cm) {
    list_base = (uint32_t)__shfl((int)list_base, cfirst);
    if (created) {
      const uint32_t local = list_base + (uint32_t)__popcll(cm & ((1ull << lane) - 1ull));
      if (local < A.mr_per)
        A.rlist[sub * A.mr_per + local] = slot;
      else
        fx_fallback(A.status, 3);
    }
  }
  if (!ok) return;
  if (WC_DBG(A.P, 16)) return;
  unsigned long long *rec = A.rec + ((size_t)(LEVEL - 1) * A.rec_cap + ridx) * kFxRecW;
  ulonglong2 *r2 = (ulonglong2 *)rec;
  r2[0] = make_ulonglong2((unsigned long long)a.n | ((unsigned long long)bin << 32), (unsigned long long)a.st);
  r2[1] = make_ulonglong2((unsigned long long)a.s[0], (unsigned long long)a.s[1]);
  r2[2] = make_ulonglong2((unsigned long long)a.s[2], (unsigned long long)a.ss[0]);
  r2[3] = make_ulonglong2((unsigned long long)a.ss[1], (unsigned long long)a.ss[2]);
  r2[4] = make_ulonglong2((unsigned long long)a.ss[3], (unsigned long long)a.ss[4]);
  r2[5] = make_ulonglong2((unsigned long long)a.ss[5], a.tmin_inv);
  r2[6] = make_ulonglong2(a.tmax_p1, (unsigned long long)old);
}

struct FxRaw {
  float x[kFxPts], y[kFxPts], z[kFxPts];
  double t[kFxPts];
};
__device__ __forceinline__ FxRaw fx_acc_load(const FxArgs &A, const uint32_t bid) {
  FxRaw r;
  const uint64_t tb = (uint64_t)bid * kFxTile, n = A.pts.n;
#pragma unroll
  for (int it = 0; it < kFxPts; ++it) {
    const uint64_t i = tb + (uint64_t)it * kFxThreads + threadIdx.x;
    r.x[it] = r.y[it] = r.z[it] = 0.f, r.t[it] = 0.0;
    if (i < n) {
      const float *f = (const float *)((const char *)A.pts.xyz + i * A.pts.xyz_stride);
      r.x[it] = f[0], r.y[it] = f[1], r.z[it] = f[2];
      r.t[it] = load_t(A.pts, i);
    }
  }
  return r;
}

template <int LEVEL>
__device__ __forceinline__ void fx_acc_body(const FxArgs &A, const uint32_t bid) {
  __shared__ unsigned long long lds_raw[kFxLds * 14];
  unsigned long long *h_key = lds_raw;
  unsigned long long(*h_rec)[13] = (unsigned long long(*)[13])(lds_raw + kFxLds);
  static_assert(kFxLds * 14 * 8 >= kFxTile * 20, "staging area fits the hash area");
  const int tid = threadIdx.x;
  const ExParams &P = A.P;
  const uint32_t sub = bid & (kFxSub - 1);
  const uint64_t n = A.pts.n;
  const uint64_t base = ((uint64_t)bid * kFxThreads + tid) * kFxPts;
  static_assert(kFxPts == 4, "the LDS transposition reads four points per lane");
  const bool direct = A.fmt == 2u && ((uint64_t)bid + 1u) * kFxTile <= n;
  FxRaw raw;
  float4 da = make_float4(0.f, 0.f, 0.f, 0.f), db = da, dc = da;
  double2 dt01 = make_double2(0.0, 0.0), dt23 = dt01;
  if (direct) {
    const float4 *xp = (const float4 *)((const char *)A.pts.xyz + base * 12u);
    const double2 *tp = (const double2 *)((const char *)A.pts.time + base * 8u);
    da = xp[0], db = xp[1], dc = xp[2];
    dt01 = tp[0], dt23 = tp[1];
  } else {
    raw = fx_acc_load(A, bid);
  }
  double x0, y0, z0;
  load_xyz(A.pts, 0, x0, y0, z0);
  int k0x = fx_vox(x0, P.vs, A.inv_vs), k0y = fx_vox(y0, P.vs, A.inv_vs), k0z = fx_vox(z0, P.vs, A.inv_vs);
  const float q0 = P.vs_f / 4;

  double px[kFxPts], py[kFxPts], pz[kFxPts], pt[kFxPts];
  if (direct) {
    const float4 a = da, b = db, c = dc;
    const double2 t01 = dt01, t23 = dt23;
    for (int i = tid; i < kFxLds * 14; i += kFxThreads) lds_raw[i] = 0ull;
    px[0] = a.x, py[0] = a.y, pz[0] = a.z, px[1] = a.w, py[1] = b.x, pz[1] = b.y;
    px[2] = b.z, py[2] = b.w, pz[2] = c.x, px[3] = c.y, py[3] = c.z, pz[3] = c.w;
    pt[0] = t01.x, pt[1] = t01.y, pt[2] = t23.x, pt[3] = t23.y;
    __syncthreads();
  } else {
    double *s_t = (double *)lds_raw;
    float *s_x = (float *)(s_t + kFxTile), *s_y = s_x + kFxTile, *s_z = s_y + kFxTile;
#pragma unroll
    for (int it = 0; it < kFxPts; ++it) {
      s_x[it * kFxThreads + tid] = raw.x[it], s_y[it * kFxThreads + tid] = raw.y[it], s_z[it * kFxThreads + tid] = raw.z[it];
      s_t[it * kFxThreads + tid] = raw.t[it];
    }
    __syncthreads();
    {
      const float4 vx = ((const float4 *)s_x)[tid], vy = ((const float4 *)s_y)[tid], vz = ((const float4 *)s_z)[tid];
      const double2 t01 = ((const double2 *)s_t)[2 * tid], t23 = ((const double2 *)s_t)[2 * tid + 1];
      px[0] = vx.x, px[1] = vx.y, px[2] = vx.z, px[3] = vx.w;
      py[0] = vy.x, py[1] = vy.y, py[2] = vy.z, py[3] = vy.w;
      pz[0] = vz.x, pz[1] = vz.y, pz[2] = vz.z, pz[3] = vz.w;
      pt[0] = t01.x, pt[1] = t01.y, pt[2] = t23.x, pt[3] = t23.y;
    }
    __syncthreads();
    for (int i = tid; i < kFxLds * 14; i += kFxThreads) lds_raw[i] = 0ull;
    __syncthreads();
  }
  if (WC_DBG(P, 4)) {
    double sacc = 0;
#pragma unroll
    for (int j = 0; j < kFxPts; ++j) sacc += px[j] + py[j] + pz[j] + pt[j];
    if (sacc == 1.2345) h_key[tid] = 1ull;
    return;
  }
  auto flush_lds = [&](unsigned long long code, const FxPart &a) -> bool {
    uint32_t s = fx_hash32((uint32_t)code ^ (uint32_t)(code >> 29)) & (kFxLds - 1);
    for (int probe = 0; probe < kFxLdsProbe; ++probe) {
      const unsigned long long old = atomicCAS(&h_key[s], 0ull, code);
      if (old == 0ull || old == code) {
        fx_add_cell(&h_rec[s][0], a);
        return true;
      }
      s = (s + 1) & (kFxLds - 1);
    }
    return false;
  };

  unsigned long long code[kFxPts];
  double tmag[kFxPts];
  uint32_t qlx[kFxPts], qly[kFxPts], qlz[kFxPts];
  bool bad_key = false, bad_time = false;
  int kxs[kFxPts], kys[kFxPts], kzs[kFxPts];
  bool fin[kFxPts];
#pragma unroll
  for (int j = 0; j < kFxPts; ++j) fin[j] = true;
  {
    bool near = false;
#pragma unroll
    for (int j = 0; j < kFxPts; ++j) {
      const double qx = px[j] * A.inv_vs, qy = py[j] * A.inv_vs, qz = pz[j] * A.inv_vs;
      const double fx = floor(qx), fy = floor(qy), fz = floor(qz);
      const double dx = qx - fx, dy = qy - fy, dz = qz - fz;
      near = near || !(dx > 1e-6 && dx < 1.0 - 1e-6) || !(dy > 1e-6 && dy < 1.0 - 1e-6) || !(dz > 1e-6 && dz < 1.0 - 1e-6);
      kxs[j] = (int)fx, kys[j] = (int)fy, kzs[j] = (int)fz;
    }
    if (__ballot(near)) {
      bool redo = false;
#pragma unroll
      for (int j = 0; j < kFxPts; ++j) {
        const double qx = px[j] * A.inv_vs, qy = py[j] * A.inv_vs, qz = pz[j] * A.inv_vs;
        const double dx = qx - floor(qx), dy = qy - floor(qy), dz = qz - floor(qz);
        fin[j] = finite3(px[j], py[j], pz[j]);
        redo = redo || (fin[j] && (!(dx > 1e-6 && dx < 1.0 - 1e-6) || !(dy > 1e-6 && dy < 1.0 - 1e-6) || !(dz > 1e-6 && dz < 1.0 - 1e-6)));
      }
      if (__ballot(redo)) {
#pragma unroll
        for (int j = 0; j < kFxPts; ++j)
          if (fin[j]) kxs[j] = fx_vox(px[j], P.vs, A.inv_vs), kys[j] = fx_vox(py[j], P.vs, A.inv_vs), kzs[j] = fx_vox(pz[j], P.vs, A.inv_vs);
      }
    }
  }
  if (!finite3(x0, y0, z0)) {
    ex_origin(A.pts, x0, y0, z0);
    k0x = fx_vox(x0, P.vs, A.inv_vs), k0y = fx_vox(y0, P.vs, A.inv_vs), k0z = fx_vox(z0, P.vs, A.inv_vs);
  }
  uint32_t split4[kFxPts], base4[kFxPts];
  if (LEVEL == 2) {
    uint32_t key1[kFxPts], slot4[kFxPts], found4[kFxPts];
    bool ok4[kFxPts];
#pragma unroll
    for (int j = 0; j < kFxPts; ++j) {
      const int rx = kxs[j] - k0x + 512, ry = kys[j] - k0y + 512, rz = kzs[j] - k0z + 512;
      ok4[j] = base + j < n && fin[j] && (unsigned)rx < 1024u && (unsigned)ry < 1024u && (unsigned)rz < 1024u;
      key1[j] = ((uint32_t)rx | ((uint32_t)ry << 10) | ((uint32_t)rz << 20)) + 1u;
      slot4[j] = fx_hash32(key1[j]) & A.tr_mask;
    }
#pragma unroll
    for (int j = 0; j < kFxPts; ++j) found4[j] = ok4[j] ? __hip_atomic_load(&A.rkey[slot4[j]], __ATOMIC_RELAXED, __HIP_MEMORY_SCOPE_AGENT) : 0u;
    const uint32_t maxprobe = A.status[kFxStMaxProbe];
    bool coll = false;
#pragma unroll
    for (int j = 0; j < kFxPts; ++j) coll = coll || (ok4[j] && found4[j] != key1[j] && (found4[j] != 0u || maxprobe != 0u));
    if (__ballot(coll)) {
#pragma unroll
      for (int j = 0; j < kFxPts; ++j)
        if (ok4[j] && found4[j] != key1[j] && (found4[j] != 0u || maxprobe != 0u)) {
          const uint32_t r = fx_root_slot(A, key1[j], 0u, false, maxprobe);
          slot4[j] = r != 0xFFFFFFFFu ? r : 0u;
          found4[j] = r != 0xFFFFFFFFu ? key1[j] : 0u;
        }
    }
#pragma unroll
    for (int j = 0; j < kFxPts; ++j) {
      const bool present = ok4[j] && found4[j] == key1[j];
      const uint32_t *h32 = (const uint32_t *)(A.blk + (size_t)(present ? slot4[j] : 0u) * kFxBlockW);
      const uint2 sb = *(const uint2 *)(h32 + 12);
      split4[j] = present ? sb.x : 0u, base4[j] = present ? sb.y : 0u;
    }
  }
#pragma unroll
  for (int j = 0; j < kFxPts; ++j) {
    const bool have = base + j < n && fin[j];
    const double x = px[j], y = py[j], z = pz[j], t = pt[j];
    const int kx = kxs[j], ky = kys[j], kz = kzs[j];
    const int rx = kx - k0x + 512, ry = ky - k0y + 512, rz = kz - k0z + 512;
    const bool key_ok = (unsigned)rx < 1024u && (unsigned)ry < 1024u && (unsigned)rz < 1024u;
    const uint32_t key = (uint32_t)rx | ((uint32_t)ry << 10) | ((uint32_t)rz << 20);
    const double cx = fma((double)kx, (double)P.vs_f, 0.5 * (double)P.vs_f), cy = fma((double)ky, (double)P.vs_f, 0.5 * (double)P.vs_f),
                 cz = fma((double)kz, (double)P.vs_f, 0.5 * (double)P.vs_f);
    const int bx = x > cx, by = y > cy, bz = z > cz;
    const uint32_t o1 = (uint32_t)(4 * bx + 2 * by + bz);
    const double trel = t - A.t_lo;
    const double tm = fma(trel, A.tick, kFxMagic);
    const bool time_ok = tm >= kFxMagic && tm < kFxMagic + 2199023255552.0;
    bad_key = bad_key || (have && !key_ok);
    bad_time = bad_time || (have && key_ok && !time_ok);
    bool use = have && key_ok && time_ok;
    const uint32_t bin = (uint32_t)(use ? trel * A.inv_w : 0.0);
    unsigned long long c;
    if (LEVEL == 1) {
      c = (unsigned long long)key | ((unsigned long long)o1 << 30) | ((unsigned long long)bin << 33) | (1ull << 63);
    } else {
      use = use && ((split4[j] >> o1) & 1u);
      const uint32_t qn = base4[j] + (uint32_t)__popc(split4[j] & ((1u << o1) - 1u));
      const double c1x = cx + (double)((float)(2 * bx - 1) * q0), c1y = cy + (double)((float)(2 * by - 1) * q0),
                   c1z = cz + (double)((float)(2 * bz - 1) * q0);
      const uint32_t o2 = (uint32_t)(4 * (x > c1x) + 2 * (y > c1y) + (z > c1z));
      c = (unsigned long long)qn | ((unsigned long long)o2 << 28) | ((unsigned long long)bin << 31) | (1ull << 63);
    }
    const double ccx = cx, ccy = cy, ccz = cz;
    code[j] = use ? c : 0ull;
    tmag[j] = tm;
    const double mx = fma(x - ccx, A.qs, kFxMagic), my = fma(y - ccy, A.qs, kFxMagic), mz = fma(z - ccz, A.qs, kFxMagic);
    qlx[j] = (uint32_t)__double_as_longlong(mx), qly[j] = (uint32_t)__double_as_longlong(my), qlz[j] = (uint32_t)__double_as_longlong(mz);
  }
  if (bad_key) raise_flag(A.status, kFlagKeyRange);
  if (bad_time) raise_flag(A.status, kFlagTimeRange);
  FxEarly early, no_early;
  no_early.key1 = 0u, no_early.s0 = 0u, no_early.found = 0u, no_early.lead = threadIdx.x & 63;
  early = no_early;
  if (LEVEL == 1) {
    unsigned long long lc = 0ull;
#pragma unroll
    for (int j = 0; j < kFxPts; ++j) lc = code[j] ? code[j] : lc;
    const uint32_t pk = lc ? (uint32_t)(lc & 0x3FFFFFFFull) + 1u : 0u;
    unsigned long long todo = __ballot(pk != 0u);
    int lead = threadIdx.x & 63, rounds = 0;
    while (todo && rounds < 4) {
      const int first = __ffsll((long long)todo) - 1;
      const uint32_t k0 = (uint32_t)__shfl((int)pk, first);
      const bool mine = pk != 0u && pk == k0;
      if (mine) lead = first;
      todo &= ~__ballot(mine);
      ++rounds;
    }
    if (!todo && !(WC_DBG(P, 64))) {
      early.key1 = pk;
      early.lead = lead;
      early.s0 = fx_hash32(pk) & A.tr_mask;
      if (pk != 0u && (int)(threadIdx.x & 63) == lead) early.found = atomicCAS(&A.rkey[early.s0], 0u, pk);
    }
  }
  const int lane = tid & 63, wave = tid >> 6;
  const unsigned long long lt_mask = (1ull << lane) - 1ull;
  bool bnd[kFxPts];
  {
    unsigned long long open = 0ull;
#pragma unroll
    for (int j = 0; j < kFxPts; ++j) {
      bnd[j] = code[j] != 0ull && open != 0ull && code[j] != open;
      if (code[j] != 0ull) open = code[j];
    }
  }
  const uint32_t rec0 = bid * (uint32_t)kFxRecTile + (uint32_t)kFxLds + (uint32_t)wave * 4u * (uint32_t)kFxDirect;
  auto close_partial = [&](int cls, bool closing, unsigned long long c, const FxPart &a) {
    const unsigned long long mclass = __ballot(closing);
    if (!mclass || (WC_DBG(P, 2))) return;
    if (__popcll(mclass) <= kFxDirect) {
      fx_push<LEVEL>(A, closing, c & 0x7FFFFFFFFFFFFFFFull, a, sub, rec0 + (uint32_t)cls * (uint32_t)kFxDirect + (uint32_t)__popcll(mclass & lt_mask), cls == 3 ? early : no_early);
    } else {
      const bool failed = closing && !flush_lds(c, a);
      const unsigned long long mf = __ballot(failed);
      if (mf) {
        const uint32_t sp = bid & 7u;
        uint32_t b0 = 0;
        if (lane == 0) b0 = atomicAdd(fx_cnt(A, kFxStSpillBank, sp), (uint32_t)__popcll(mf));
        b0 = (uint32_t)__shfl((int)b0, 0);
        const uint32_t k = b0 + (uint32_t)__popcll(mf & lt_mask);
        const bool room = k < A.spill_per;
        if (failed && !room) fx_fallback(A.status, 4);
        fx_push<LEVEL>(A, failed && room, c & 0x7FFFFFFFFFFFFFFFull, a, sub, A.rec_tiles * (uint32_t)kFxRecTile + sp * A.spill_per + k, no_early);
      }
    }
  };

  FxPart acc;
  double tlo_m = 0.0, thi_m = 0.0;
  uint32_t nfix = 0;
  auto raw_zero = [&]() {
    fx_zero(acc);
    tlo_m = 1.0e300, thi_m = 0.0;
    nfix = 0;
  };
  auto fx_fix = [&]() {
    const uint32_t dn = acc.n - nfix;
    nfix = acc.n;
    const unsigned long long c1 = (unsigned long long)(dn * kFxMagicHi) << 32, c2 = (unsigned long long)(dn * kFxMagic2Hi) << 32;
    acc.st = (long long)((unsigned long long)acc.st - c1);
#pragma unroll
    for (int i = 0; i < 3; ++i) acc.s[i] = (long long)((unsigned long long)acc.s[i] - c1);
#pragma unroll
    for (int i = 0; i < 6; ++i) acc.ss[i] = (long long)((unsigned long long)acc.ss[i] - c2);
    const unsigned long long lo = (unsigned long long)__double_as_longlong(tlo_m) - kFxMagicBits, hi = (unsigned long long)__double_as_longlong(thi_m) - kFxMagicBits;
    acc.tmin_inv = acc.n ? kFxTMax - lo : 0ull;
    acc.tmax_p1 = acc.n ? hi + 1ull : 0ull;
  };
  raw_zero();
  unsigned long long cur = 0ull;
#pragma unroll
  for (int j = 0; j < kFxPts; ++j) {
    if (j) {
      if (__ballot(bnd[j])) {
        fx_fix();
        close_partial(j - 1, bnd[j], cur, acc);
      }
      if (bnd[j]) raw_zero();
    }
    if (code[j] == 0ull) continue;
    cur = code[j];
    acc.n += 1;
    acc.st += __double_as_longlong(tmag[j]);
    const long long bx = (long long)(((unsigned long long)(kFxMagicHi - (qlx[j] >> 31)) << 32) | qlx[j]);
    const long long by = (long long)(((unsigned long long)(kFxMagicHi - (qly[j] >> 31)) << 32) | qly[j]);
    const long long bz = (long long)(((unsigned long long)(kFxMagicHi - (qlz[j] >> 31)) << 32) | qlz[j]);
    acc.s[0] += bx, acc.s[1] += by, acc.s[2] += bz;
    const double x = __longlong_as_double(bx) - kFxMagic, y = __longlong_as_double(by) - kFxMagic, z = __longlong_as_double(bz) - kFxMagic;
    acc.ss[0] += __double_as_longlong(fma(x, x, kFxMagic2)), acc.ss[1] += __double_as_longlong(fma(x, y, kFxMagic2));
    acc.ss[2] += __double_as_longlong(fma(x, z, kFxMagic2)), acc.ss[3] += __double_as_longlong(fma(y, y, kFxMagic2));
    acc.ss[4] += __double_as_longlong(fma(y, z, kFxMagic2)), acc.ss[5] += __double_as_longlong(fma(z, z, kFxMagic2));
    tlo_m = fmin(tlo_m, tmag[j]), thi_m = fmax(thi_m, tmag[j]);
  }
  fx_fix();
  bool e_made = false;
  unsigned long long e_cm = 0ull;
  uint32_t e_base = 0;
  if (LEVEL == 1) {
    e_made = early.key1 != 0u && (int)(threadIdx.x & 63) == early.lead && early.found == 0u;
    e_cm = __ballot(e_made);
    if (e_cm && (int)(threadIdx.x & 63) == __ffsll((long long)e_cm) - 1) e_base = atomicAdd(fx_cnt(A, kFxStRoots, sub), (uint32_t)__popcll(e_cm));
  }
  {
    const unsigned long long mycode = acc.n ? cur : 0ull;
    auto shr32 = [](uint32_t v, auto dtag) -> uint32_t {
      constexpr int d = decltype(dtag)::value;
      return (uint32_t)__builtin_amdgcn_update_dpp(0, (int)v, 0x110 + d, 0xF, 0xF, true);
    };
    auto shr64 = [&](unsigned long long v, auto dtag) -> unsigned long long {
      return (unsigned long long)shr32((uint32_t)v, dtag) | ((unsigned long long)shr32((uint32_t)(v >> 32), dtag) << 32);
    };
    const int rl = lane & 15;
    const unsigned long long prevc = shr64(mycode, std::integral_constant<int, 1>{});
    uint32_t head = (rl == 0 || prevc != mycode) ? 1u : 0u;
    auto step = [&](auto dtag) {
      constexpr int d = decltype(dtag)::value;
      if (!__ballot(rl >= d && !head)) return;
      const uint32_t ohead = shr32(head, dtag);
      const uint32_t on = shr32(acc.n, dtag);
      const long long ost = (long long)shr64((unsigned long long)acc.st, dtag);
      long long os[3], oss[6];
#pragma unroll
      for (int i = 0; i < 3; ++i) os[i] = (long long)shr64((unsigned long long)acc.s[i], dtag);
#pragma unroll
      for (int i = 0; i < 6; ++i) oss[i] = (long long)shr64((unsigned long long)acc.ss[i], dtag);
      const unsigned long long omin = shr64(acc.tmin_inv, dtag), omax = shr64(acc.tmax_p1, dtag);
      if (rl >= d && !head) {
        acc.n += on, acc.st += ost;
#pragma unroll
        for (int i = 0; i < 3; ++i) acc.s[i] += os[i];
#pragma unroll
        for (int i = 0; i < 6; ++i) acc.ss[i] += oss[i];
        acc.tmin_inv = max(acc.tmin_inv, omin);
        acc.tmax_p1 = max(acc.tmax_p1, omax);
        head = ohead;
      }
    };
    step(std::integral_constant<int, 1>{});
    step(std::integral_constant<int, 2>{});
    step(std::integral_constant<int, 4>{});
    step(std::integral_constant<int, 8>{});
    const uint32_t nlo = (uint32_t)__builtin_amdgcn_update_dpp(0, (int)(uint32_t)mycode, 0x101, 0xF, 0xF, true);
    const uint32_t nhi = (uint32_t)__builtin_amdgcn_update_dpp(0, (int)(uint32_t)(mycode >> 32), 0x101, 0xF, 0xF, true);
    const unsigned long long nextc = (unsigned long long)nlo | ((unsigned long long)nhi << 32);
    const bool tail = mycode != 0ull && (rl == 15 || nextc != mycode);
    close_partial(3, tail, mycode, acc);
  }
  __syncthreads();
  if (WC_DBG(P, 1)) return;
  static_assert(kFxLds == kFxThreads, "one hash cell per thread in the final loop");
  {
    const int i = tid;
    const unsigned long long c = h_key[i];
    FxPart a;
    fx_zero(a);
    if (c != 0ull) {
      a.n = (uint32_t)h_rec[i][0];
      a.st = (long long)h_rec[i][1];
      for (int w = 0; w < 3; ++w) a.s[w] = (long long)h_rec[i][2 + w];
      for (int w = 0; w < 6; ++w) a.ss[w] = (long long)h_rec[i][5 + w];
      a.tmin_inv = h_rec[i][11];
      a.tmax_p1 = h_rec[i][12];
    }
    if (__ballot(c != 0ull)) fx_push<LEVEL>(A, c != 0ull, c & 0x7FFFFFFFFFFFFFFFull, a, sub, bid * (uint32_t)kFxRecTile + (uint32_t)i, no_early);
  }
  if (LEVEL == 1 && e_cm) {
    const int l = threadIdx.x & 63;
    const uint32_t list_base = (uint32_t)__shfl((int)e_base, __ffsll((long long)e_cm) - 1);
    if (e_made) {
      const uint32_t local = list_base + (uint32_t)__popcll(e_cm & ((1ull << l) - 1ull));
      if (local < A.mr_per)
        A.rlist[sub * A.mr_per + local] = early.s0;
      else
        fx_fallback(A.status, 5);
    }
  }
}

template <int LEVEL>
__global__ void __launch_bounds__(kFxThreads) k_fx_acc(FxArgs A) {
  fx_acc_body<LEVEL>(A, blockIdx.x);
}

struct FxBatch {
  const FxArgs *args;
  const uint32_t *start;
  const uint32_t *flags;
  int K;
};
__device__ __forceinline__ int fx_batch_find(const FxBatch &B, uint32_t b, uint32_t &local) {
  int k = 0;
  while (k + 1 < B.K && b >= B.start[k + 1]) ++k;
  local = b - B.start[k];
  return k;
}
#define WC_FX_BATCH_ARGS(sA, B, k)                                                                 \
  __shared__ FxArgs sA;                                                                            \
  static_assert(sizeof(FxArgs) % 8 == 0, "copied as 64-bit words");                                 \
  for (uint32_t w_ = threadIdx.x; w_ < sizeof(FxArgs) / 8; w_ += blockDim.x)                      \
    ((unsigned long long *)&sA)[w_] = ((const unsigned long long *)&(B).args[k])[w_];              \
  __syncthreads();
template <int LEVEL>
__global__ void __launch_bounds__(kFxThreads) k_fx_acc_b(FxBatch B) {
  uint32_t bid;
  const int k = fx_batch_find(B, blockIdx.x, bid);
  if (LEVEL == 2 && !(B.flags[k] & 1u)) return;
  WC_FX_BATCH_ARGS(sA, B, k)
  fx_acc_body<LEVEL>(sA, bid);
}

template <int LEVEL>
__device__ __forceinline__ void fx_merge_body(const FxArgs &A, const uint32_t bid, const uint32_t nblk) {
  const uint32_t bank = LEVEL == 1 ? kFxStRoots : kFxStNodes2;
  const uint32_t per = LEVEL == 1 ? A.mr_per : A.mq_per;
  uint32_t total = 0, cnts[kFxSub];
#pragma unroll
  for (int j = 0; j < kFxSub; ++j) {
    cnts[j] = min(*fx_cnt(A, bank, j), per);
    total += cnts[j];
  }
  for (uint32_t gi = bid; gi < total; gi += nblk) {
    uint32_t pidx = 0, rem = gi;
    bool found = false;
#pragma unroll
    for (int j = 0; j < kFxSub; ++j) {
      if (!found) {
        if (rem < cnts[j]) {
          pidx = (uint32_t)j * per + rem;
          found = true;
        } else {
          rem -= cnts[j];
        }
      }
    }
    if (LEVEL == 1) pidx = A.rlist[pidx];
    const unsigned long long *blk = (LEVEL == 1 ? A.blk : A.blk2) + (size_t)pidx * kFxBlockW;
    const uint32_t head = ((const uint32_t *)(blk + kFxHdrW))[threadIdx.x];
    if (head == 0u) continue;
    unsigned long long *first = A.rec + ((size_t)(LEVEL - 1) * A.rec_cap + (head - 1u)) * kFxRecW;
    ulonglong2 *f2 = (ulonglong2 *)first;
    const ulonglong2 w0 = f2[0], w6 = f2[6];
    uint32_t idx = (uint32_t)w6.y;
    if (idx == 0u) continue;
    const ulonglong2 w1 = f2[1], w2 = f2[2], w3 = f2[3], w4 = f2[4], w5 = f2[5];
    const uint32_t bin = (uint32_t)(w0.x >> 32);
    FxPart b;
    b.n = (uint32_t)w0.x, b.st = (long long)w0.y;
    b.s[0] = (long long)w1.x, b.s[1] = (long long)w1.y, b.s[2] = (long long)w2.x;
    b.ss[0] = (long long)w2.y, b.ss[1] = (long long)w3.x, b.ss[2] = (long long)w3.y;
    b.ss[3] = (long long)w4.x, b.ss[4] = (long long)w4.y, b.ss[5] = (long long)w5.x;
    b.tmin_inv = w5.y, b.tmax_p1 = w6.x;
    bool same = true;
    int guard = 0;
    for (; idx != 0u && guard < 100000; ++guard) {
      const ulonglong2 *r2 = (const ulonglong2 *)(A.rec + ((size_t)(LEVEL - 1) * A.rec_cap + (idx - 1u)) * kFxRecW);
      const ulonglong2 v0 = r2[0], v1 = r2[1], v2 = r2[2], v3 = r2[3], v4 = r2[4], v5 = r2[5], v6 = r2[6];
      same = same && (uint32_t)(v0.x >> 32) == bin;
      b.n += (uint32_t)v0.x, b.st += (long long)v0.y;
      b.s[0] += (long long)v1.x, b.s[1] += (long long)v1.y, b.s[2] += (long long)v2.x;
      b.ss[0] += (long long)v2.y, b.ss[1] += (long long)v3.x, b.ss[2] += (long long)v3.y;
      b.ss[3] += (long long)v4.x, b.ss[4] += (long long)v4.y, b.ss[5] += (long long)v5.x;
      b.tmin_inv = max(b.tmin_inv, v5.y), b.tmax_p1 = max(b.tmax_p1, v6.x);
      idx = (uint32_t)v6.y;
    }
    if (guard >= A.P.merge_min) {
      uint32_t *hm = host_mailbox(A.status);
      if (hm) hm[LEVEL == 1 ? 15 : 16] = 1u;
    }
    if (!same || idx != 0u) continue;
    f2[0] = make_ulonglong2((unsigned long long)b.n | ((unsigned long long)bin << 32), (unsigned long long)b.st);
    f2[1] = make_ulonglong2((unsigned long long)b.s[0], (unsigned long long)b.s[1]);
    f2[2] = make_ulonglong2((unsigned long long)b.s[2], (unsigned long long)b.ss[0]);
    f2[3] = make_ulonglong2((unsigned long long)b.ss[1], (unsigned long long)b.ss[2]);
    f2[4] = make_ulonglong2((unsigned long long)b.ss[3], (unsigned long long)b.ss[4]);
    f2[5] = make_ulonglong2((unsigned long long)b.ss[5], b.tmin_inv);
    f2[6] = make_ulonglong2(b.tmax_p1, 0ull);
  }
}

template <int LEVEL>
__global__ void __launch_bounds__(128) k_fx_merge(FxArgs A) {
  fx_merge_body<LEVEL>(A, blockIdx.x, gridDim.x);
}
template <int LEVEL>
__global__ void __launch_bounds__(128) k_fx_merge_b(FxBatch B) {
  uint32_t bid;
  const int k = fx_batch_find(B, blockIdx.x, bid);
  if (!(B.flags[k] & 2u) || (LEVEL == 2 && !(B.flags[k] & 1u))) return;
  WC_FX_BATCH_ARGS(sA, B, k)
  fx_merge_body<LEVEL>(sA, bid, B.start[k + 1] - B.start[k]);
}

__device__ __forceinline__ long long fx_gsum8(long long v) {
  for (int m = 1; m < 8; m <<= 1) v += __shfl_xor(v, m, 8);
  return v;
}
__device__ __forceinline__ void fx_gsum8(FxPart &a) {
  a.n = (uint32_t)fx_gsum8((long long)a.n);
  a.st = fx_gsum8(a.st);
  for (int i = 0; i < 3; ++i) a.s[i] = fx_gsum8(a.s[i]);
  for (int i = 0; i < 6; ++i) a.ss[i] = fx_gsum8(a.ss[i]);
}

#include "fx_eig3.h"

struct FxPca {
  Pca r;
  bool near;
  int which;
};

__device__ __forceinline__ void fx_pca(const FxArgs &A, const FxPart &m, const double *cc, FxPca &o) {
  const double n = (double)m.n;
  const double in = fx_rcp(n), iq = A.inv_q * in, iqq = A.inv_qq * in;
  const double mx = (double)m.s[0] * iq, my = (double)m.s[1] * iq, mz = (double)m.s[2] * iq;
  wc::M3 C;
  C.m[0][0] = (double)m.ss[0] * iqq - mx * mx;
  C.m[0][1] = C.m[1][0] = (double)m.ss[1] * iqq - mx * my;
  C.m[0][2] = C.m[2][0] = (double)m.ss[2] * iqq - mx * mz;
  C.m[1][1] = (double)m.ss[3] * iqq - my * my;
  C.m[1][2] = C.m[2][1] = (double)m.ss[4] * iqq - my * mz;
  C.m[2][2] = (double)m.ss[5] * iqq - mz * mz;
  Pca &r = o.r;
  r.c[0] = cc[0] + mx, r.c[1] = cc[1] + my, r.c[2] = cc[2] + mz;
  r.tmean = A.t_lo + ((double)m.st * in) * A.inv_tick;
  wc::M3 V;
  fx_eig3(C, r.ev, V);
  for (int i = 0; i < 3; ++i) {
    r.nrm[i] = V.m[i][0];
    for (int j = 0; j < 3; ++j) r.cov[3 * i + j] = C.m[i][j];
  }
  const double sum = (r.ev[0] + r.ev[1]) + r.ev[2];
  const double isum = fx_rcp(sum);
  r.like = 2 * (r.ev[1] - r.ev[0]) * isum;
  const double R2 = r.c[0] * r.c[0] + r.c[1] * r.c[1] + r.c[2] * r.c[2] + 1.0;
  const double dl = 16.0 * (n * fx_rsqrt(n)) * R2 * 1.1102230246251565e-16 + A.band0;
  const double dlike = 6.0 * dl * fabs(isum) + 1e-13;
  o.near = (fabs(r.ev[0] - A.P.thr) <= dl) || (fabs(r.like - A.P.min_like) <= dlike) || !(sum > 0.0);
  o.which = (fabs(r.ev[0] - A.P.thr) <= dl) ? 0 : ((fabs(r.like - A.P.min_like) <= dlike) ? 1 : 2);
}

__device__ __forceinline__ bool fx_surely_not_plane(const FxArgs &A, const FxPart &m, const double *cc) {
  const double n = (double)m.n;
  const double in = fx_rcp(n), iq = A.inv_q * in, iqq = A.inv_qq * in;
  const double mx = (double)m.s[0] * iq, my = (double)m.s[1] * iq, mz = (double)m.s[2] * iq;
  const double c00 = (double)m.ss[0] * iqq - mx * mx, c01 = (double)m.ss[1] * iqq - mx * my, c02 = (double)m.ss[2] * iqq - mx * mz;
  const double c11 = (double)m.ss[3] * iqq - my * my, c12 = (double)m.ss[4] * iqq - my * mz, c22 = (double)m.ss[5] * iqq - mz * mz;
  const double det = c00 * (c11 * c22 - c12 * c12) - c01 * (c01 * c22 - c12 * c02) + c02 * (c01 * c12 - c11 * c02);
  const double tr = (c00 + c11) + c22;
  const double px = cc[0] + mx, py = cc[1] + my, pz = cc[2] + mz;
  const double R2 = px * px + py * py + pz * pz + 1.0;
  const double dl = 16.0 * (n * fx_rsqrt(n)) * R2 * 1.1102230246251565e-16 + A.band0;
  return m.n != 0u && tr > 0.0 && 4.0 * det > 1.001 * (A.P.thr + dl) * tr * tr;
}

struct FxEmit {
  uint64_t entry;
  uint32_t bkt, r, rank;
  int lead;
  bool on;
};
__device__ __forceinline__ void fx_emit_end(const FxArgs &A, const FxEmit &e) {
  const uint32_t r = (uint32_t)__shfl((int)e.r, e.lead) + e.rank;
  if (e.on && r < A.slot_bin_cap) A.slot_bins[(size_t)e.bkt * A.slot_bin_cap + r] = e.entry;
}
__device__ __forceinline__ FxEmit fx_emit_begin(const FxArgs &A, const Pca &rr, uint32_t slot, int layer, uint32_t o1, uint32_t o2, uint32_t ord, int kx,
                                                int ky, int kz, float q0) {
  const ExParams &P = A.P;
  double nx = rr.nrm[0], ny = rr.nrm[1], nz = rr.nrm[2];
  const double d = nx * (rr.c[0] - P.view[0]) + ny * (rr.c[1] - P.view[1]) + nz * (rr.c[2] - P.view[2]);
  if (d < 0) nx = -nx, ny = -ny, nz = -nz;
  const float ql = layer == 0 ? q0 : (layer == 1 ? q0 / 2 : (q0 / 2) / 2);
  wc_surfel sf;
  sf.t = rr.tmean;
  sf.center[0] = rr.c[0], sf.center[1] = rr.c[1], sf.center[2] = rr.c[2];
  for (int i = 0; i < 9; ++i) sf.cov[i] = rr.cov[i];
  sf.normal[0] = nx, sf.normal[1] = ny, sf.normal[2] = nz;
  sf.resolution = (double)(ql * 4);
  sf.sigma = sqrt(rr.ev[0]);
  A.slots[slot] = sf;
  uint32_t node = (uint32_t)layer;
  if (layer >= 1) node |= o1 << 2;
  if (layer == 2) node |= o2 << 5;
  A.slot_ids[slot] = wc_surfel_id{kx, ky, kz, node | (ord << 8)};
  const double frac = (rr.tmean - A.t_lo) * A.inv_span;
  if (!(frac >= 0.0 && frac <= 1.0)) raise_flag(A.status, kFlagTimeRange);
  const uint64_t key = (uint64_t)min(max(frac, 0.0) * 4294967296.0, 4294967295.0);
  FxEmit e;
  e.on = true;
  e.bkt = (uint32_t)(key >> 20);
  e.entry = (key << 32) | (uint64_t)slot;
  const int lane = threadIdx.x & 63;
  e.lead = lane, e.rank = 0;
  uint32_t gsize = 1;
  if (!(WC_DBG(P, 16384))) {
    unsigned long long todo = __ballot(true);
    for (int round = 0; todo && round < 4; ++round) {
      const int lead = __ffsll((long long)todo) - 1;
      const uint32_t b0 = (uint32_t)__shfl((int)e.bkt, lead);
      const bool mine = e.bkt == b0;
      const unsigned long long m = __ballot(mine);
      if (mine) e.lead = lead, e.rank = (uint32_t)__popcll(m & ((1ull << lane) - 1ull)), gsize = (uint32_t)__popcll(m);
      todo &= ~m;
    }
  }
  e.r = 0;
  if (e.lead == lane) e.r = atomicAdd(&A.slot_counts[e.bkt], gsize);
  return e;
}
__device__ __forceinline__ void fx_emit(const FxArgs &A, const Pca &rr, uint32_t slot, int layer, uint32_t o1, uint32_t o2, uint32_t ord, int kx,
                                        int ky, int kz, float q0) {
  fx_emit_end(A, fx_emit_begin(A, rr, slot, layer, o1, o2, ord, kx, ky, kz, q0));
}

constexpr int kFxChains = 4;
constexpr int kFxJobCap = 512;
constexpr int kFxJobW = 12;
template <int N, int CAP = kFxChains>
__device__ __forceinline__ void fx_stepn(const FxArgs &A, int level, uint32_t (&ix)[CAP], const uint32_t (&bin)[CAP], FxPart (&b)[CAP]) {
  const unsigned long long *base = A.rec + (size_t)(level - 1) * A.rec_cap * kFxRecW;
  ulonglong2 w[N][7];
#pragma unroll
  for (int j = 0; j < N; ++j) {
    const ulonglong2 *r2 = (const ulonglong2 *)(base + (size_t)(ix[j] ? ix[j] - 1u : 0u) * kFxRecW);
#pragma unroll
    for (int i = 0; i < 7; ++i) w[j][i] = r2[i];
  }
#pragma unroll
  for (int j = 0; j < N; ++j) {
    const bool on = ix[j] != 0u;
    const unsigned long long m = on ? ~0ull : 0ull;
    if (on && (uint32_t)(w[j][0].x >> 32) != bin[j]) fx_fallback(A.status, 6);
    FxPart &q = b[j];
    q.n += (uint32_t)(w[j][0].x & m);
    q.st += (long long)(w[j][0].y & m);
    q.s[0] += (long long)(w[j][1].x & m), q.s[1] += (long long)(w[j][1].y & m), q.s[2] += (long long)(w[j][2].x & m);
    q.ss[0] += (long long)(w[j][2].y & m), q.ss[1] += (long long)(w[j][3].x & m), q.ss[2] += (long long)(w[j][3].y & m);
    q.ss[3] += (long long)(w[j][4].x & m), q.ss[4] += (long long)(w[j][4].y & m), q.ss[5] += (long long)(w[j][5].x & m);
    q.tmin_inv = max(q.tmin_inv, w[j][5].y & m);
    q.tmax_p1 = max(q.tmax_p1, w[j][6].x & m);
    ix[j] = (uint32_t)(w[j][6].y & m);
  }
}

struct FxWhy {
  int gap;
  int slots;
  int jobs;
  int walk1;
  int walkn;
  int big_bin;
  int job_which;
};

template <int LEVEL>
__device__ __forceinline__ uint32_t fx_dense_parent(const FxArgs &A, const uint32_t (&cnts)[kFxSub], uint32_t per, uint32_t gi, bool have_parent) {
  uint32_t pidx = 0;
  if (have_parent) {
    uint32_t rem = gi;
    bool found = false;
#pragma unroll
    for (int j = 0; j < kFxSub; ++j) {
      const uint32_t cj = cnts[j];
      if (!found) {
        if (rem < cj) {
          pidx = (uint32_t)j * per + rem;
          found = true;
        } else {
          rem -= cj;
        }
      }
    }
  }
  if (LEVEL == 1 && have_parent) pidx = A.rlist[pidx];
  return pidx;
}

template <int LEVEL>
__device__ __forceinline__ void fx_parent_header(const FxArgs &A, const unsigned long long *blk, uint32_t pidx, bool have_parent, uint32_t &key,
                                                 uint32_t &o1p, uint32_t &minbin) {
  const uint32_t *h32 = (const uint32_t *)blk;
  key = 0, o1p = 0, minbin = 0;
  if (have_parent) {
    minbin = 0xFFFFFFFFu - h32[2];
    if (LEVEL == 1) {
      key = A.rkey[pidx] - 1u;
    } else {
      const uint32_t ro = h32[0];
      o1p = (ro >> 28) & 7u;
      key = h32[1] - 1u;
    }
  }
}

__device__ __forceinline__ void fx_key_voxel(const ExParams &P, uint32_t key, int k0x, int k0y, int k0z, int &kx, int &ky, int &kz, double (&cc)[3]) {
  kx = (int)(key & 1023u) - 512 + k0x, ky = (int)((key >> 10) & 1023u) - 512 + k0y, kz = (int)(key >> 20) - 512 + k0z;
  cc[0] = (0.5 + kx) * P.vs_f, cc[1] = (0.5 + ky) * P.vs_f, cc[2] = (0.5 + kz) * P.vs_f;
}

__device__ __forceinline__ uint32_t fx_load_heads(const unsigned long long *blk, bool have_parent, uint32_t minbin, uint32_t *heads) {
  uint32_t occ = 0;
  const uint4 *hq = (const uint4 *)(blk + kFxHdrW) + (threadIdx.x & 7) * (kFxSlots / 4);
  uint32_t hv[kFxSlots];
#pragma unroll
  for (int q = 0; q < kFxSlots / 4; ++q) {
    const uint4 v = have_parent ? hq[q] : make_uint4(0u, 0u, 0u, 0u);
    hv[4 * q] = v.x, hv[4 * q + 1] = v.y, hv[4 * q + 2] = v.z, hv[4 * q + 3] = v.w;
  }
#pragma unroll
  for (int s = 0; s < kFxSlots; ++s) {
    const uint32_t p = ((uint32_t)s - minbin) & (kFxSlots - 1);
// ... 455 lines not shown
```

Measured before the change: 21290 Mpts/s.

## Split fx push into claim/link/store and add selectable accumulation forms

Breaks the per-partial push into a hash-slot claim, a list-head link, and a record store. This lets the accumulation kernel issue all directly routed slot claims and links early, before the per-cell sums are finished, so atomic latency overlaps with the reduction. It replaces the old single early-claim path. It also adds a staged-rounds form that computes point codes into LDS, plus a dev option and A/B script to pick between forms. The default form links early with rounds at level 1. The extra code paths add register pressure and more template instantiations.

Measured after the change: 21920 Mpts/s (median of 6 runs). 1.03x the previous value.

```diff
diff --git a/profiles/dev/ab_acc_forms.py b/profiles/dev/ab_acc_forms.py
--- /dev/null
+++ b/profiles/dev/ab_acc_forms.py
@@ -0,0 +1,58 @@
+import json, os, sys, time
+sys.path.insert(0, os.path.join(os.path.dirname(os.path.abspath(__file__)), "..", "..", "wildcat-slam_amd", "python"))
+import numpy as np
+from wildcat_slam_amd import lib, synth
+from wildcat_slam_amd import records as Rec
+
+which = sys.argv[1] if len(sys.argv) > 1 else "c2"
+alts = int(sys.argv[2]) if len(sys.argv) > 2 else 5
+steps = int(sys.argv[3]) if len(sys.argv) > 3 else 200
+out = sys.argv[4] if len(sys.argv) > 4 else None
+pts = {"c2": lambda: synth.g2_lattice(3906, m=32)[0], "c2soa": lambda: synth.g2_lattice(3906, m=32)[0], "c5": lambda: synth.g2_lattice(39062, m=32)[0],
+       "room": lambda: synth.g1_room(1_000_000, seed=synth.SEED + 3)}[which]()
+n = len(pts)
+cap = (3 * n) // 20 + 1
+ctx = lib.Context(0)
+d_out, d_ids = ctx.alloc(cap * 144), ctx.alloc(cap * 16)
+if which.endswith("soa"):
+    d_xyz = ctx.to_device(np.stack([pts["x"], pts["y"], pts["z"]], axis=1).astype(np.float32).reshape(-1))
+    d_t = ctx.to_device(np.ascontiguousarray(pts["time"], np.float64))
+    desc = Rec.Points(d_xyz.ptr, d_t.ptr, 12, 8, n)
+else:
+    d = ctx.to_device(pts)
+    desc = ctx.points_desc(d, n)
+t_lo, t_hi = float(pts["time"][0]), float(pts["time"][-1])
+enqueue, finish = ctx.prepare_extract(desc, d_out, d_ids, cap, t_lo, t_hi)
+FORMS = (0, 1, 2, -1)
+wall = {f: [] for f in FORMS}
+acc = {f: [] for f in FORMS}
+nodes = {f: [] for f in FORMS}
+for a in range(alts):
+    for f in FORMS:
+        ctx.set_dev_option("fx_acc_form", f)
+        for _ in range(20):
+            enqueue(), finish()
+        ctx.sync()
+        t0 = time.perf_counter()
+        for _ in range(steps):
+            enqueue(), finish()
+        ctx.sync()
+        wall[f].append(round((time.perf_counter() - t0) / steps * 1e3, 5))
+        ctx.extract_profile(True)
+        v, w = [], []
+        for _ in range(24):
+            enqueue(), finish()
+            st = ctx.extract_stage_ms()
+            v.append(st["point_sort"]), w.append(st["roots_stream"])
+        ctx.extract_profile(False)
+        acc[f].append(round(1e3 * float(np.median(v[4:])), 2))
+        nodes[f].append(round(1e3 * float(np.median(w[4:])), 2))
+res = dict(workload=which, points=n, alternations=alts, sweeps=steps, assert_fast=ctx.extract_path_info()["fast"],
+           wall_ms={str(f): wall[f] for f in FORMS}, k_fx_acc_us={str(f): acc[f] for f in FORMS}, k_fx_nodes_us={str(f): nodes[f] for f in FORMS})
+for f in FORMS:
+    print("form %2d: wall ms %s  [%.5f .. %.5f]   k_fx_acc us %s   k_fx_nodes us %s" % (f, wall[f], min(wall[f]), max(wall[f]), acc[f], nodes[f]))
+print(json.dumps(res))
+if out:
+    with open(out, "w") as fh:
+        json.dump(res, fh, indent=1)
+ctx.close()
diff --git a/wildcat-slam_amd/csrc/ctx.h b/wildcat-slam_amd/csrc/ctx.h
--- a/wildcat-slam_amd/csrc/ctx.h
+++ b/wildcat-slam_amd/csrc/ctx.h
@@ -31,6 +31,7 @@
   int debug_skip = 0;
   int fx_merge_min = 3;
   int fx_split = -1;
+  int fx_acc_form = -1;
   int no_bucket_sort = 0;
   int ex_sync = 0;
   int match_pair_serial = 0;
diff --git a/wildcat-slam_amd/csrc/ctx.hip b/wildcat-slam_amd/csrc/ctx.hip
--- a/wildcat-slam_amd/csrc/ctx.hip
+++ b/wildcat-slam_amd/csrc/ctx.hip
@@ -60,6 +60,7 @@
     {"debug_skip", "WC_DEBUG_SKIP", &wc_dev_opts::debug_skip, false},
     {"fx_merge_min", "WC_FX_MERGE_MIN", &wc_dev_opts::fx_merge_min, false},
     {"fx_split", "WC_FX_SPLIT", &wc_dev_opts::fx_split, false},
+    {"fx_acc_form", "WC_FX_ACC_FORM", &wc_dev_opts::fx_acc_form, false},
     {"no_bucket_sort", "WC_NO_BUCKET_SORT", &wc_dev_opts::no_bucket_sort, true},
     {"ex_sync", "WC_EX_SYNC", &wc_dev_opts::ex_sync, true},
     {"match_pair_serial", "WC_MATCH_PAIR_SERIAL", &wc_dev_opts::match_pair_serial, true},
diff --git a/wildcat-slam_amd/csrc/extract.hip b/wildcat-slam_amd/csrc/extract.hip
--- a/wildcat-slam_amd/csrc/extract.hip
+++ b/wildcat-slam_amd/csrc/extract.hip
@@ -1805,7 +1805,7 @@
     ctx->ex.deferred = true;
     return WC_OK;
   }
-  k_fx_acc<1><<<tiles, kFxThreads, 0, st>>>(A);
+  fx_launch_acc<1>(ctx, tiles, st, A);
   dbg_sync("k_fx_acc<1>");
   ex_mark(ctx, 2);
   if (M.fx_long_lists) k_fx_merge<1><<<std::min<unsigned>(ngrid * 2u, 8192u), 128, 0, st>>>(A);
@@ -1832,7 +1832,7 @@
   std::memcpy(&A, ctx->ex.roots_args, sizeof(A));
   ExMemory &M = ctx->ex_mem;
   if (layer2) {
-    k_fx_acc<2><<<ex_fx_tiles(A.pts.n), kFxThreads, 0, st>>>(A);
+    fx_launch_acc<2>(ctx, ex_fx_tiles(A.pts.n), st, A);
     if (M.fx_long_lists2) k_fx_merge<2><<<std::min(8192u, std::max(64u, M.last_splits)), 128, 0, st>>>(A);
     const unsigned g2 = ex_fx_layer2_grid(ex_fx_node_grid(A.pts.n), M.last_splits);
     if (ctx->ex.fx_split) {
@@ -2198,14 +2198,14 @@
   FxBatch B;
   B.args = (const FxArgs *)d, B.K = Kd, B.flags = dt + 3 * (K + 1);
   B.start = dt;
-  k_fx_acc_b<1><<<s_acc[Kd], kFxThreads, 0, st>>>(B);
+  fx_launch_acc_b<1>(ctx, s_acc[Kd], st, B);
   B.start = dt + (K + 1);
   if (any_merge) k_fx_merge_b<1><<<s_nodes[Kd], 128, 0, st>>>(B);
   k_fx_walk_b<1><<<s_nodes[Kd], 64, 0, st>>>(B);
   k_fx_test_b<1><<<s_nodes[Kd], 64, 0, st>>>(B);
   if (any_l2) {
     B.start = dt;
-    k_fx_acc_b<2><<<s_acc[Kd], kFxThreads, 0, st>>>(B);
+    fx_launch_acc_b<2>(ctx, s_acc[Kd], st, B);
     B.start = dt + 2 * (K + 1);
     if (any_merge) k_fx_merge_b<2><<<s_g2[Kd], 128, 0, st>>>(B);
     k_fx_walk_b<2><<<s_g2[Kd], 64, 0, st>>>(B);
diff --git a/wildcat-slam_amd/csrc/extract_fast.inc b/wildcat-slam_amd/csrc/extract_fast.inc
--- a/wildcat-slam_amd/csrc/extract_fast.inc
+++ b/wildcat-slam_amd/csrc/extract_fast.inc
@@ -129,16 +129,12 @@
   atomicMax(&cell[12], a.tmax_p1);
 }
 
-struct FxEarly {
-  uint32_t key1, s0, found;
+struct FxClaim {
   int lead;
+  uint32_t gmb, s0, found;
 };
 template <int LEVEL>
-__device__ __forceinline__ void fx_push(const FxArgs &A, bool active, unsigned long long code, const FxPart &a, uint32_t sub, uint32_t ridx,
-                                        const FxEarly &E) {
-  const int lane = threadIdx.x & 63;
-  unsigned long long *blk = nullptr;
-  uint32_t oct, bin, pkey;
+__device__ __forceinline__ void fx_code_fields(unsigned long long code, uint32_t &pkey, uint32_t &oct, uint32_t &bin) {
   if (LEVEL == 1) {
     pkey = (uint32_t)(code & 0x3FFFFFFFull) + 1u;
     oct = (uint32_t)(code >> 30) & 7u;
@@ -148,6 +144,12 @@
     oct = (uint32_t)(code >> 28) & 7u;
     bin = (uint32_t)(code >> 31) & 0xFFFFFu;
   }
+}
+template <int LEVEL>
+__device__ __forceinline__ FxClaim fx_link_claim(const FxArgs &A, bool active, unsigned long long code) {
+  const int lane = threadIdx.x & 63;
+  uint32_t oct, bin, pkey;
+  fx_code_fields<LEVEL>(code, pkey, oct, bin);
   int lead = lane;
   uint32_t gmb = bin;
   {
@@ -162,27 +164,36 @@
       todo &= ~__ballot(mine);
     }
   }
+  FxClaim c;
+  c.lead = lead, c.gmb = gmb, c.s0 = 0u, c.found = 0u;
+  if (LEVEL == 1) {
+    c.s0 = fx_hash32(pkey) & A.tr_mask;
+    if (active && lane == lead && !(WC_DBG(A.P, 64))) c.found = atomicCAS(&A.rkey[c.s0], 0u, pkey);
+  }
+  return c;
+}
+template <int LEVEL>
+__device__ __forceinline__ bool fx_link_head(const FxArgs &A, bool active, unsigned long long code, uint32_t sub, uint32_t ridx, const FxClaim &c,
+                                             uint32_t &old) {
+  const int lane = threadIdx.x & 63;
+  unsigned long long *blk = nullptr;
+  uint32_t oct, bin, pkey;
+  fx_code_fields<LEVEL>(code, pkey, oct, bin);
+  const int lead = c.lead;
+  const uint32_t gmb = c.gmb;
   const bool leader = active && lane == lead;
   uint32_t slot = 0xFFFFFFFFu;
   bool created = false;
-  const uint32_t e_found = (uint32_t)__shfl((int)E.found, E.lead);
-  const bool e_have = LEVEL == 1 && E.key1 != 0u && E.key1 == pkey;
   if (leader) {
     if (LEVEL == 1) {
       if (WC_DBG(A.P, 64)) {
-        slot = fx_hash32(pkey) & A.tr_mask;
+        slot = c.s0;
+      } else if (c.found == 0u || c.found == pkey) {
+        slot = c.s0;
+        created = c.found == 0u;
       } else {
-        uint32_t s = fx_hash32(pkey) & A.tr_mask;
-        int probe = 0;
-        if (e_have) {
-          if (e_found == 0u || e_found == pkey) {
-            slot = s;
-          } else {
-            s = (s + 1u) & A.tr_mask;
-            probe = 1;
-          }
-        }
-        for (; slot == 0xFFFFFFFFu && probe < 64; ++probe) {
+        uint32_t s = (c.s0 + 1u) & A.tr_mask;
+        for (int probe = 1; probe < 64; ++probe) {
           const uint32_t k = atomicCAS(&A.rkey[s], 0u, pkey);
           if (k == 0u || k == pkey) {
             slot = s;
@@ -207,7 +218,7 @@
     atomicMax((uint32_t *)b0 + 2, 0xFFFFFFFFu - gmb);
   }
   const uint32_t myslot = (uint32_t)__shfl((int)slot, lead);
-  uint32_t old = 0;
+  old = 0u;
   const bool ok = active && myslot != 0xFFFFFFFFu;
   if (ok) {
     blk = (LEVEL == 1 ? A.blk : A.blk2) + (size_t)myslot * kFxBlockW;
@@ -224,8 +235,13 @@
         fx_fallback(A.status, 3);
     }
   }
-  if (!ok) return;
+  return ok;
+}
+template <int LEVEL>
+__device__ __forceinline__ void fx_store(const FxArgs &A, unsigned long long code, const FxPart &a, uint32_t ridx, uint32_t old) {
   if (WC_DBG(A.P, 16)) return;
+  uint32_t oct, bin, pkey;
+  fx_code_fields<LEVEL>(code, pkey, oct, bin);
   unsigned long long *rec = A.rec + ((size_t)(LEVEL - 1) * A.rec_cap + ridx) * kFxRecW;
   ulonglong2 *r2 = (ulonglong2 *)rec;
   r2[0] = make_ulonglong2((unsigned long long)a.n | ((unsigned long long)bin << 32), (unsigned long long)a.st);
@@ -236,11 +252,86 @@
   r2[5] = make_ulonglong2((unsigned long long)a.ss[5], a.tmin_inv);
   r2[6] = make_ulonglong2(a.tmax_p1, (unsigned long long)old);
 }
+template <int LEVEL>
+__device__ __forceinline__ void fx_push(const FxArgs &A, bool active, unsigned long long code, const FxPart &a, uint32_t sub, uint32_t ridx) {
+  const FxClaim c = fx_link_claim<LEVEL>(A, active, code);
+  uint32_t old;
+  if (fx_link_head<LEVEL>(A, active, code, sub, ridx, c, old)) fx_store<LEVEL>(A, code, a, ridx, old);
+}
+
+struct FxPt {
+  unsigned long long code;
+  double tmag;
+  uint32_t qlx, qly, qlz;
+};
+__device__ __forceinline__ bool fx_pt_index(const FxArgs &A, double x, double y, double z, int &kx, int &ky, int &kz) {
+  const double qx = x * A.inv_vs, qy = y * A.inv_vs, qz = z * A.inv_vs;
+  const double fx = floor(qx), fy = floor(qy), fz = floor(qz);
+  const double dx = qx - fx, dy = qy - fy, dz = qz - fz;
+  const bool near = !(dx > 1e-6 && dx < 1.0 - 1e-6) || !(dy > 1e-6 && dy < 1.0 - 1e-6) || !(dz > 1e-6 && dz < 1.0 - 1e-6);
+  kx = (int)fx, ky = (int)fy, kz = (int)fz;
+  bool fin = true;
+  if (__ballot(near)) {
+    fin = finite3(x, y, z);
+    if (__ballot(fin && near)) {
+      if (fin) kx = fx_vox(x, A.P.vs, A.inv_vs), ky = fx_vox(y, A.P.vs, A.inv_vs), kz = fx_vox(z, A.P.vs, A.inv_vs);
+    }
+  }
+  return fin;
+}
+__device__ __forceinline__ bool fx_pt_key(int kx, int ky, int kz, int k0x, int k0y, int k0z, uint32_t &key) {
+  const int rx = kx - k0x + 512, ry = ky - k0y + 512, rz = kz - k0z + 512;
+  key = (uint32_t)rx | ((uint32_t)ry << 10) | ((uint32_t)rz << 20);
+  return (unsigned)rx < 1024u && (unsigned)ry < 1024u && (unsigned)rz < 1024u;
+}
+template <int LEVEL>
+__device__ __forceinline__ FxPt fx_pt_code(const FxArgs &A, bool have, double x, double y, double z, double t, int kx, int ky, int kz, int k0x,
+                                           int k0y, int k0z, uint32_t split, uint32_t base2, bool &bad_key, bool &bad_time) {
+  const ExParams &P = A.P;
+  uint32_t key;
+  const bool key_ok = fx_pt_key(kx, ky, kz, k0x, k0y, k0z, key);
+  const double cx = fma((double)kx, (double)P.vs_f, 0.5 * (double)P.vs_f), cy = fma((double)ky, (double)P.vs_f, 0.5 * (double)P.vs_f),
+               cz = fma((double)kz, (double)P.vs_f, 0.5 * (double)P.vs_f);
+  const int bx = x > cx, by = y > cy, bz = z > cz;
+  const uint32_t o1 = (uint32_t)(4 * bx + 2 * by + bz);
+  const double trel = t - A.t_lo;
+  const double tm = fma(trel, A.tick, kFxMagic);
+  const bool time_ok = tm >= kFxMagic && tm < kFxMagic + 2199023255552.0;
+  bad_key = bad_key || (have && !key_ok);
+  bad_time = bad_time || (have && key_ok && !time_ok);
+  bool use = have && key_ok && time_ok;
+  const uint32_t bin = (uint32_t)(use ? trel * A.inv_w : 0.0);
+  unsigned long long c;
+  if (LEVEL == 1) {
+    c = (unsigned long long)key | ((unsigned long long)o1 << 30) | ((unsigned long long)bin << 33) | (1ull << 63);
+  } else {
+    const float q0 = P.vs_f / 4;
+    use = use && ((split >> o1) & 1u);
+    const uint32_t qn = base2 + (uint32_t)__popc(split & ((1u << o1) - 1u));
+    const double c1x = cx + (double)((float)(2 * bx - 1) * q0), c1y = cy + (double)((float)(2 * by - 1) * q0),
+                 c1z = cz + (double)((float)(2 * bz - 1) * q0);
+    const uint32_t o2 = (uint32_t)(4 * (x > c1x) + 2 * (y > c1y) + (z > c1z));
+    c = (unsigned long long)qn | ((unsigned long long)o2 << 28) | ((unsigned long long)bin << 31) | (1ull << 63);
+  }
+  FxPt o;
+  o.code = use ? c : 0ull;
+  o.tmag = tm;
+  const double mx = fma(x - cx, A.qs, kFxMagic), my = fma(y - cy, A.qs, kFxMagic), mz = fma(z - cz, A.qs, kFxMagic);
+  o.qlx = (uint32_t)__double_as_longlong(mx), o.qly = (uint32_t)__double_as_longlong(my), o.qlz = (uint32_t)__double_as_longlong(mz);
+  return o;
+}
+__device__ __forceinline__ FxPt fx_point(const FxArgs &A, bool in_range, double x, double y, double z, double t, int k0x, int k0y, int k0z,
+                                         bool &bad_key, bool &bad_time) {
+  int kx, ky, kz;
+  const bool fin = fx_pt_index(A, x, y, z, kx, ky, kz);
+  return fx_pt_code<1>(A, in_range && fin, x, y, z, t, kx, ky, kz, k0x, k0y, k0z, 0u, 0u, bad_key, bad_time);
+}
 
 struct FxRaw {
   float x[kFxPts], y[kFxPts], z[kFxPts];
   double t[kFxPts];
 };
+template <bool FULL = false>
 __device__ __forceinline__ FxRaw fx_acc_load(const FxArgs &A, const uint32_t bid) {
   FxRaw r;
   const uint64_t tb = (uint64_t)bid * kFxTile, n = A.pts.n;
@@ -248,17 +339,20 @@
   for (int it = 0; it < kFxPts; ++it) {
     const uint64_t i = tb + (uint64_t)it * kFxThreads + threadIdx.x;
     r.x[it] = r.y[it] = r.z[it] = 0.f, r.t[it] = 0.0;
-    if (i < n) {
+    if (FULL || i < n) {
       const float *f = (const float *)((const char *)A.pts.xyz + i * A.pts.xyz_stride);
       r.x[it] = f[0], r.y[it] = f[1], r.z[it] = f[2];
       r.t[it] = load_t(A.pts, i);
     }
+    if (FULL) __builtin_amdgcn_sched_barrier(0);
   }
   return r;
 }
 
-template <int LEVEL>
+constexpr int kFxAccForm = 3;
+template <int LEVEL, int FORM>
 __device__ __forceinline__ void fx_acc_body(const FxArgs &A, const uint32_t bid) {
+  constexpr bool kRounds = LEVEL == 1 && (FORM & 1) != 0, kLinkEarly = (FORM & 2) != 0;
   __shared__ unsigned long long lds_raw[kFxLds * 14];
   unsigned long long *h_key = lds_raw;
   unsigned long long(*h_rec)[13] = (unsigned long long(*)[13])(lds_raw + kFxLds);
@@ -269,7 +363,58 @@
   const uint64_t n = A.pts.n;
   const uint64_t base = ((uint64_t)bid * kFxThreads + tid) * kFxPts;
   static_assert(kFxPts == 4, "the LDS transposition reads four points per lane");
-  const bool direct = A.fmt == 2u && ((uint64_t)bid + 1u) * kFxTile <= n;
+  const bool full = ((uint64_t)bid + 1u) * kFxTile <= n;
+  const bool direct = A.fmt == 2u && full;
+  unsigned long long code[kFxPts];
+  double tmag[kFxPts];
+  uint32_t qlx[kFxPts], qly[kFxPts], qlz[kFxPts];
+  bool bad_key = false, bad_time = false;
+  if (kRounds && !direct) {
+    static_assert(kFxTile * 28 == kFxLds * 14 * 8, "the staged results fill the hash area exactly");
+    unsigned long long *s_code = lds_raw;
+    double *s_tm = (double *)(lds_raw + kFxTile);
+    uint32_t *s_qx = (uint32_t *)(lds_raw + 2 * kFxTile), *s_qy = s_qx + kFxTile, *s_qz = s_qy + kFxTile;
+    double x0, y0, z0;
+    load_xyz(A.pts, 0, x0, y0, z0);
+    auto rounds = [&](auto full_tag) -> bool {
+      constexpr bool kFull = decltype(full_tag)::value;
+      const FxRaw raw = fx_acc_load<kFull>(A, bid);
+      if (!finite3(x0, y0, z0)) ex_origin(A.pts, x0, y0, z0);
+      const int k0x = fx_vox(x0, P.vs, A.inv_vs), k0y = fx_vox(y0, P.vs, A.inv_vs), k0z = fx_vox(z0, P.vs, A.inv_vs);
+      if (WC_DBG(P, 4)) {
+        double sacc = 0;
+#pragma unroll
+        for (int j = 0; j < kFxPts; ++j) sacc += (double)raw.x[j] + (double)raw.y[j] + (double)raw.z[j] + raw.t[j];
+        if (sacc == 1.2345) h_key[tid] = 1ull;
+        return false;
+      }
+      const uint64_t tb = (uint64_t)bid * kFxTile;
+#pragma unroll
+      for (int it = 0; it < kFxPts; ++it) {
+        const uint32_t i = (uint32_t)it * kFxThreads + (uint32_t)tid;
+        const FxPt p = fx_point(A, kFull || tb + i < n, (double)raw.x[it], (double)raw.y[it], (double)raw.z[it], raw.t[it], k0x, k0y, k0z, bad_key,
+                                bad_time);
+        s_code[i] = p.code, s_tm[i] = p.tmag;
+        s_qx[i] = p.qlx, s_qy[i] = p.qly, s_qz[i] = p.qlz;
+      }
+      return true;
+    };
+    if (!(full ? rounds(std::true_type{}) : rounds(std::false_type{}))) return;
+    __syncthreads();
+    {
+      const ulonglong2 c01 = ((const ulonglong2 *)s_code)[2 * tid], c23 = ((const ulonglong2 *)s_code)[2 * tid + 1];
+      const double2 t01 = ((const double2 *)s_tm)[2 * tid], t23 = ((const double2 *)s_tm)[2 * tid + 1];
+      const uint4 vx = ((const uint4 *)s_qx)[tid], vy = ((const uint4 *)s_qy)[tid], vz = ((const uint4 *)s_qz)[tid];
+      code[0] = c01.x, code[1] = c01.y, code[2] = c23.x, code[3] = c23.y;
+      tmag[0] = t01.x, tmag[1] = t01.y, tmag[2] = t23.x, tmag[3] = t23.y;
+      qlx[0] = vx.x, qlx[1] = vx.y, qlx[2] = vx.z, qlx[3] = vx.w;
+      qly[0] = vy.x, qly[1] = vy.y, qly[2] = vy.z, qly[3] = vy.w;
+      qlz[0] = vz.x, qlz[1] = vz.y, qlz[2] = vz.z, qlz[3] = vz.w;
+    }
+    __syncthreads();
+    for (int i = tid; i < kFxLds * 14; i += kFxThreads) lds_raw[i] = 0ull;
+    __syncthreads();
+  } else {
   FxRaw raw;
   float4 da = make_float4(0.f, 0.f, 0.f, 0.f), db = da, dc = da;
   double2 dt01 = make_double2(0.0, 0.0), dt23 = dt01;
@@ -284,7 +429,6 @@
   double x0, y0, z0;
   load_xyz(A.pts, 0, x0, y0, z0);
   int k0x = fx_vox(x0, P.vs, A.inv_vs), k0y = fx_vox(y0, P.vs, A.inv_vs), k0z = fx_vox(z0, P.vs, A.inv_vs);
-  const float q0 = P.vs_f / 4;
 
   double px[kFxPts], py[kFxPts], pz[kFxPts], pt[kFxPts];
   if (direct) {
@@ -323,6 +467,61 @@
     if (sacc == 1.2345) h_key[tid] = 1ull;
     return;
   }
+  int kxs[kFxPts], kys[kFxPts], kzs[kFxPts];
+  bool fin[kFxPts];
+#pragma unroll
+  for (int j = 0; j < kFxPts; ++j) fin[j] = fx_pt_index(A, px[j], py[j], pz[j], kxs[j], kys[j], kzs[j]);
+  if (!finite3(x0, y0, z0)) {
+    ex_origin(A.pts, x0, y0, z0);
+    k0x = fx_vox(x0, P.vs, A.inv_vs), k0y = fx_vox(y0, P.vs, A.inv_vs), k0z = fx_vox(z0, P.vs, A.inv_vs);
+  }
+  uint32_t split4[kFxPts], base4[kFxPts];
+#pragma unroll
+  for (int j = 0; j < kFxPts; ++j) split4[j] = base4[j] = 0u;
+  if (LEVEL == 2) {
+    uint32_t key1[kFxPts], slot4[kFxPts], found4[kFxPts];
+    bool ok4[kFxPts];
+#pragma unroll
+    for (int j = 0; j < kFxPts; ++j) {
+      uint32_t key;
+      const bool key_ok = fx_pt_key(kxs[j], kys[j], kzs[j], k0x, k0y, k0z, key);
+      ok4[j] = base + j < n && fin[j] && key_ok;
+      key1[j] = key + 1u;
+      slot4[j] = fx_hash32(key1[j]) & A.tr_mask;
+    }
+#pragma unroll
+    for (int j = 0; j < kFxPts; ++j) found4[j] = ok4[j] ? __hip_atomic_load(&A.rkey[slot4[j]], __ATOMIC_RELAXED, __HIP_MEMORY_SCOPE_AGENT) : 0u;
+    const uint32_t maxprobe = A.status[kFxStMaxProbe];
+    bool coll = false;
+#pragma unroll
+    for (int j = 0; j < kFxPts; ++j) coll = coll || (ok4[j] && found4[j] != key1[j] && (found4[j] != 0u || maxprobe != 0u));
+    if (__ballot(coll)) {
+#pragma unroll
+      for (int j = 0; j < kFxPts; ++j)
+        if (ok4[j] && found4[j] != key1[j] && (found4[j] != 0u || maxprobe != 0u)) {
+          const uint32_t r = fx_root_slot(A, key1[j], 0u, false, maxprobe);
+          slot4[j] = r != 0xFFFFFFFFu ? r : 0u;
+          found4[j] = r != 0xFFFFFFFFu ? key1[j] : 0u;
+        }
+    }
+#pragma unroll
+    for (int j = 0; j < kFxPts; ++j) {
+      const bool present = ok4[j] && found4[j] == key1[j];
+      const uint32_t *h32 = (const uint32_t *)(A.blk + (size_t)(present ? slot4[j] : 0u) * kFxBlockW);
+      const uint2 sb = *(const uint2 *)(h32 + 12);
+      split4[j] = present ? sb.x : 0u, base4[j] = present ? sb.y : 0u;
+    }
+  }
+#pragma unroll
+  for (int j = 0; j < kFxPts; ++j) {
+    const FxPt p = fx_pt_code<LEVEL>(A, base + j < n && fin[j], px[j], py[j], pz[j], pt[j], kxs[j], kys[j], kzs[j], k0x, k0y, k0z, split4[j], base4[j],
+                                     bad_key, bad_time);
+    code[j] = p.code, tmag[j] = p.tmag;
+    qlx[j] = p.qlx, qly[j] = p.qly, qlz[j] = p.qlz;
+  }
+  }
+  if (bad_key) raise_flag(A.status, kFlagKeyRange);
+  if (bad_time) raise_flag(A.status, kFlagTimeRange);
   auto flush_lds = [&](unsigned long long code, const FxPart &a) -> bool {
     uint32_t s = fx_hash32((uint32_t)code ^ (uint32_t)(code >> 29)) & (kFxLds - 1);
     for (int probe = 0; probe < kFxLdsProbe; ++probe) {
@@ -336,158 +535,63 @@
     return false;
   };
 
-  unsigned long long code[kFxPts];
-  double tmag[kFxPts];
-  uint32_t qlx[kFxPts], qly[kFxPts], qlz[kFxPts];
-  bool bad_key = false, bad_time = false;
-  int kxs[kFxPts], kys[kFxPts], kzs[kFxPts];
-  bool fin[kFxPts];
-#pragma unroll
-  for (int j = 0; j < kFxPts; ++j) fin[j] = true;
-  {
-    bool near = false;
-#pragma unroll
-    for (int j = 0; j < kFxPts; ++j) {
-      const double qx = px[j] * A.inv_vs, qy = py[j] * A.inv_vs, qz = pz[j] * A.inv_vs;
-      const double fx = floor(qx), fy = floor(qy), fz = floor(qz);
-      const double dx = qx - fx, dy = qy - fy, dz = qz - fz;
-      near = near || !(dx > 1e-6 && dx < 1.0 - 1e-6) || !(dy > 1e-6 && dy < 1.0 - 1e-6) || !(dz > 1e-6 && dz < 1.0 - 1e-6);
-      kxs[j] = (int)fx, kys[j] = (int)fy, kzs[j] = (int)fz;
-    }
-    if (__ballot(near)) {
-      bool redo = false;
-#pragma unroll
-      for (int j = 0; j < kFxPts; ++j) {
-        const double qx = px[j] * A.inv_vs, qy = py[j] * A.inv_vs, qz = pz[j] * A.inv_vs;
-        const double dx = qx - floor(qx), dy = qy - floor(qy), dz = qz - floor(qz);
-        fin[j] = finite3(px[j], py[j], pz[j]);
-        redo = redo || (fin[j] && (!(dx > 1e-6 && dx < 1.0 - 1e-6) || !(dy > 1e-6 && dy < 1.0 - 1e-6) || !(dz > 1e-6 && dz < 1.0 - 1e-6)));
-      }
-      if (__ballot(redo)) {
-#pragma unroll
-        for (int j = 0; j < kFxPts; ++j)
-          if (fin[j]) kxs[j] = fx_vox(px[j], P.vs, A.inv_vs), kys[j] = fx_vox(py[j], P.vs, A.inv_vs), kzs[j] = fx_vox(pz[j], P.vs, A.inv_vs);
-      }
-    }
-  }
-  if (!finite3(x0, y0, z0)) {
-    ex_origin(A.pts, x0, y0, z0);
-    k0x = fx_vox(x0, P.vs, A.inv_vs), k0y = fx_vox(y0, P.vs, A.inv_vs), k0z = fx_vox(z0, P.vs, A.inv_vs);
-  }
-  uint32_t split4[kFxPts], base4[kFxPts];
-  if (LEVEL == 2) {
-    uint32_t key1[kFxPts], slot4[kFxPts], found4[kFxPts];
-    bool ok4[kFxPts];
-#pragma unroll
-    for (int j = 0; j < kFxPts; ++j) {
-      const int rx = kxs[j] - k0x + 512, ry = kys[j] - k0y + 512, rz = kzs[j] - k0z + 512;
-      ok4[j] = base + j < n && fin[j] && (unsigned)rx < 1024u && (unsigned)ry < 1024u && (unsigned)rz < 1024u;
-      key1[j] = ((uint32_t)rx | ((uint32_t)ry << 10) | ((uint32_t)rz << 20)) + 1u;
-      slot4[j] = fx_hash32(key1[j]) & A.tr_mask;
-    }
-#pragma unroll
-    for (int j = 0; j < kFxPts; ++j) found4[j] = ok4[j] ? __hip_atomic_load(&A.rkey[slot4[j]], __ATOMIC_RELAXED, __HIP_MEMORY_SCOPE_AGENT) : 0u;
-    const uint32_t maxprobe = A.status[kFxStMaxProbe];
-    bool coll = false;
-#pragma unroll
-    for (int j = 0; j < kFxPts; ++j) coll = coll || (ok4[j] && found4[j] != key1[j] && (found4[j] != 0u || maxprobe != 0u));
-    if (__ballot(coll)) {
-#pragma unroll
-      for (int j = 0; j < kFxPts; ++j)
-        if (ok4[j] && found4[j] != key1[j] && (found4[j] != 0u || maxprobe != 0u)) {
-          const uint32_t r = fx_root_slot(A, key1[j], 0u, false, maxprobe);
-          slot4[j] = r != 0xFFFFFFFFu ? r : 0u;
-          found4[j] = r != 0xFFFFFFFFu ? key1[j] : 0u;
-        }
-    }
-#pragma unroll
-    for (int j = 0; j < kFxPts; ++j) {
-      const bool present = ok4[j] && found4[j] == key1[j];
-      const uint32_t *h32 = (const uint32_t *)(A.blk + (size_t)(present ? slot4[j] : 0u) * kFxBlockW);
-      const uint2 sb = *(const uint2 *)(h32 + 12);
-      split4[j] = present ? sb.x : 0u, base4[j] = present ? sb.y : 0u;
-    }
-  }
-#pragma unroll
-  for (int j = 0; j < kFxPts; ++j) {
-    const bool have = base + j < n && fin[j];
-    const double x = px[j], y = py[j], z = pz[j], t = pt[j];
-    const int kx = kxs[j], ky = kys[j], kz = kzs[j];
-    const int rx = kx - k0x + 512, ry = ky - k0y + 512, rz = kz - k0z + 512;
-    const bool key_ok = (unsigned)rx < 1024u && (unsigned)ry < 1024u && (unsigned)rz < 1024u;
-    const uint32_t key = (uint32_t)rx | ((uint32_t)ry << 10) | ((uint32_t)rz << 20);
-    const double cx = fma((double)kx, (double)P.vs_f, 0.5 * (double)P.vs_f), cy = fma((double)ky, (double)P.vs_f, 0.5 * (double)P.vs_f),
-                 cz = fma((double)kz, (double)P.vs_f, 0.5 * (double)P.vs_f);
-    const int bx = x > cx, by = y > cy, bz = z > cz;
-    const uint32_t o1 = (uint32_t)(4 * bx + 2 * by + bz);
-    const double trel = t - A.t_lo;
-    const double tm = fma(trel, A.tick, kFxMagic);
-    const bool time_ok = tm >= kFxMagic && tm < kFxMagic + 2199023255552.0;
-    bad_key = bad_key || (have && !key_ok);
-    bad_time = bad_time || (have && key_ok && !time_ok);
-    bool use = have && key_ok && time_ok;
-    const uint32_t bin = (uint32_t)(use ? trel * A.inv_w : 0.0);
-    unsigned long long c;
-    if (LEVEL == 1) {
-      c = (unsigned long long)key | ((unsigned long long)o1 << 30) | ((unsigned long long)bin << 33) | (1ull << 63);
-    } else {
-      use = use && ((split4[j] >> o1) & 1u);
-      const uint32_t qn = base4[j] + (uint32_t)__popc(split4[j] & ((1u << o1) - 1u));
-      const double c1x = cx + (double)((float)(2 * bx - 1) * q0), c1y = cy + (double)((float)(2 * by - 1) * q0),
-                   c1z = cz + (double)((float)(2 * bz - 1) * q0);
-      const uint32_t o2 = (uint32_t)(4 * (x > c1x) + 2 * (y > c1y) + (z > c1z));
-      c = (unsigned long long)qn | ((unsigned long long)o2 << 28) | ((unsigned long long)bin << 31) | (1ull << 63);
-    }
-    const double ccx = cx, ccy = cy, ccz = cz;
-    code[j] = use ? c : 0ull;
-    tmag[j] = tm;
-    const double mx = fma(x - ccx, A.qs, kFxMagic), my = fma(y - ccy, A.qs, kFxMagic), mz = fma(z - ccz, A.qs, kFxMagic);
-    qlx[j] = (uint32_t)__double_as_longlong(mx), qly[j] = (uint32_t)__double_as_longlong(my), qlz[j] = (uint32_t)__double_as_longlong(mz);
-  }
-  if (bad_key) raise_flag(A.status, kFlagKeyRange);
-  if (bad_time) raise_flag(A.status, kFlagTimeRange);
-  FxEarly early, no_early;
-  no_early.key1 = 0u, no_early.s0 = 0u, no_early.found = 0u, no_early.lead = threadIdx.x & 63;
-  early = no_early;
-  if (LEVEL == 1) {
-    unsigned long long lc = 0ull;
-#pragma unroll
-    for (int j = 0; j < kFxPts; ++j) lc = code[j] ? code[j] : lc;
-    const uint32_t pk = lc ? (uint32_t)(lc & 0x3FFFFFFFull) + 1u : 0u;
-    unsigned long long todo = __ballot(pk != 0u);
-    int lead = threadIdx.x & 63, rounds = 0;
-    while (todo && rounds < 4) {
-      const int first = __ffsll((long long)todo) - 1;
-      const uint32_t k0 = (uint32_t)__shfl((int)pk, first);
-      const bool mine = pk != 0u && pk == k0;
-      if (mine) lead = first;
-      todo &= ~__ballot(mine);
-      ++rounds;
-    }
-    if (!todo && !(WC_DBG(P, 64))) {
-      early.key1 = pk;
-      early.lead = lead;
-      early.s0 = fx_hash32(pk) & A.tr_mask;
-      if (pk != 0u && (int)(threadIdx.x & 63) == lead) early.found = atomicCAS(&A.rkey[early.s0], 0u, pk);
-    }
-  }
   const int lane = tid & 63, wave = tid >> 6;
   const unsigned long long lt_mask = (1ull << lane) - 1ull;
   bool bnd[kFxPts];
+  unsigned long long ccode[kFxPts];
   {
     unsigned long long open = 0ull;
 #pragma unroll
     for (int j = 0; j < kFxPts; ++j) {
       bnd[j] = code[j] != 0ull && open != 0ull && code[j] != open;
+      if (j) ccode[j - 1] = open;
       if (code[j] != 0ull) open = code[j];
     }
+    ccode[kFxPts - 1] = open;
+  }
+  bool tail;
+  {
+    const unsigned long long mycode = ccode[kFxPts - 1];
+    const uint32_t nlo = (uint32_t)__builtin_amdgcn_update_dpp(0, (int)(uint32_t)mycode, 0x101, 0xF, 0xF, true);
+    const uint32_t nhi = (uint32_t)__builtin_amdgcn_update_dpp(0, (int)(uint32_t)(mycode >> 32), 0x101, 0xF, 0xF, true);
+    const unsigned long long nextc = (unsigned long long)nlo | ((unsigned long long)nhi << 32);
+    tail = mycode != 0ull && ((lane & 15) == 15 || nextc != mycode);
   }
   const uint32_t rec0 = bid * (uint32_t)kFxRecTile + (uint32_t)kFxLds + (uint32_t)wave * 4u * (uint32_t)kFxDirect;
+  auto direct_ridx = [&](int cls, unsigned long long mclass) -> uint32_t {
+    return rec0 + (uint32_t)cls * (uint32_t)kFxDirect + (uint32_t)__popcll(mclass & lt_mask);
+  };
+  auto direct_route = [](unsigned long long mclass) -> bool { return __popcll(mclass) <= kFxDirect; };
+  uint32_t l_old[kFxPts];
+  bool l_ok[kFxPts];
+#pragma unroll
+  for (int cls = 0; cls < kFxPts; ++cls) l_old[cls] = 0u, l_ok[cls] = false;
+  if (kLinkEarly && !(WC_DBG(P, 2))) {
+    FxClaim claim[kFxPts];
+#pragma unroll
+    for (int cls = 0; cls < kFxPts; ++cls) {
+      const bool closing = cls < 3 ? bnd[cls + 1] : tail;
+      const unsigned long long mclass = __ballot(closing);
+      if (mclass && direct_route(mclass)) claim[cls] = fx_link_claim<LEVEL>(A, closing, ccode[cls] & 0x7FFFFFFFFFFFFFFFull);
+    }
+#pragma unroll
+    for (int cls = 0; cls < kFxPts; ++cls) {
+      const bool closing = cls < 3 ? bnd[cls + 1] : tail;
+      const unsigned long long mclass = __ballot(closing);
+      if (mclass && direct_route(mclass))
+        l_ok[cls] = fx_link_head<LEVEL>(A, closing, ccode[cls] & 0x7FFFFFFFFFFFFFFFull, sub, direct_ridx(cls, mclass), claim[cls], l_old[cls]);
+    }
+  }
   auto close_partial = [&](int cls, bool closing, unsigned long long c, const FxPart &a) {
     const unsigned long long mclass = __ballot(closing);
     if (!mclass || (WC_DBG(P, 2))) return;
-    if (__popcll(mclass) <= kFxDirect) {
-      fx_push<LEVEL>(A, closing, c & 0x7FFFFFFFFFFFFFFFull, a, sub, rec0 + (uint32_t)cls * (uint32_t)kFxDirect + (uint32_t)__popcll(mclass & lt_mask), cls == 3 ? early : no_early);
+    if (direct_route(mclass)) {
+      const uint32_t ridx = direct_ridx(cls, mclass);
+      if (kLinkEarly) {
+        if (closing && l_ok[cls]) fx_store<LEVEL>(A, c & 0x7FFFFFFFFFFFFFFFull, a, ridx, l_old[cls]);
+      } else {
+        fx_push<LEVEL>(A, closing, c & 0x7FFFFFFFFFFFFFFFull, a, sub, ridx);
+      }
     } else {
       const bool failed = closing && !flush_lds(c, a);
       const unsigned long long mf = __ballot(failed);
@@ -499,7 +603,7 @@
         const uint32_t k = b0 + (uint32_t)__popcll(mf & lt_mask);
         const bool room = k < A.spill_per;
         if (failed && !room) fx_fallback(A.status, 4);
-        fx_push<LEVEL>(A, failed && room, c & 0x7FFFFFFFFFFFFFFFull, a, sub, A.rec_tiles * (uint32_t)kFxRecTile + sp * A.spill_per + k, no_early);
+        fx_push<LEVEL>(A, failed && room, c & 0x7FFFFFFFFFFFFFFFull, a, sub, A.rec_tiles * (uint32_t)kFxRecTile + sp * A.spill_per + k);
       }
     }
   };
@@ -551,14 +655,6 @@
     tlo_m = fmin(tlo_m, tmag[j]), thi_m = fmax(thi_m, tmag[j]);
   }
   fx_fix();
-  bool e_made = false;
-  unsigned long long e_cm = 0ull;
-  uint32_t e_base = 0;
-  if (LEVEL == 1) {
-    e_made = early.key1 != 0u && (int)(threadIdx.x & 63) == early.lead && early.found == 0u;
-    e_cm = __ballot(e_made);
-    if (e_cm && (int)(threadIdx.x & 63) == __ffsll((long long)e_cm) - 1) e_base = atomicAdd(fx_cnt(A, kFxStRoots, sub), (uint32_t)__popcll(e_cm));
-  }
   {
     const unsigned long long mycode = acc.n ? cur : 0ull;
     auto shr32 = [](uint32_t v, auto dtag) -> uint32_t {
@@ -598,10 +694,6 @@
     step(std::integral_constant<int, 2>{});
     step(std::integral_constant<int, 4>{});
     step(std::integral_constant<int, 8>{});
-    const uint32_t nlo = (uint32_t)__builtin_amdgcn_update_dpp(0, (int)(uint32_t)mycode, 0x101, 0xF, 0xF, true);
-    const uint32_t nhi = (uint32_t)__builtin_amdgcn_update_dpp(0, (int)(uint32_t)(mycode >> 32), 0x101, 0xF, 0xF, true);
-    const unsigned long long nextc = (unsigned long long)nlo | ((unsigned long long)nhi << 32);
-    const bool tail = mycode != 0ull && (rl == 15 || nextc != mycode);
     close_partial(3, tail, mycode, acc);
   }
   __syncthreads();
@@ -620,24 +712,17 @@
       a.tmin_inv = h_rec[i][11];
       a.tmax_p1 = h_rec[i][12];
     }
-    if (__ballot(c != 0ull)) fx_push<LEVEL>(A, c != 0ull, c & 0x7FFFFFFFFFFFFFFFull, a, sub, bid * (uint32_t)kFxRecTile + (uint32_t)i, no_early);
-  }
-  if (LEVEL == 1 && e_cm) {
-    const int l = threadIdx.x & 63;
-    const uint32_t list_base = (uint32_t)__shfl((int)e_base, __ffsll((long long)e_cm) - 1);
-    if (e_made) {
-      const uint32_t local = list_base + (uint32_t)__popcll(e_cm & ((1ull << l) - 1ull));
-      if (local < A.mr_per)
-        A.rlist[sub * A.mr_per + local] = early.s0;
-      else
-        fx_fallback(A.status, 5);
-    }
+    if (__ballot(c != 0ull)) fx_push<LEVEL>(A, c != 0ull, c & 0x7FFFFFFFFFFFFFFFull, a, sub, bid * (uint32_t)kFxRecTile + (uint32_t)i);
   }
 }
 
 template <int LEVEL>
 __global__ void __launch_bounds__(kFxThreads) k_fx_acc(FxArgs A) {
-  fx_acc_body<LEVEL>(A, blockIdx.x);
+  fx_acc_body<LEVEL, kFxAccForm>(A, blockIdx.x);
+}
+template <int LEVEL, int FORM>
+__global__ void __launch_bounds__(kFxThreads) k_fx_acc_form(FxArgs A) {
+  fx_acc_body<LEVEL, FORM>(A, blockIdx.x);
 }
 
 struct FxBatch {
@@ -664,7 +749,42 @@
   const int k = fx_batch_find(B, blockIdx.x, bid);
   if (LEVEL == 2 && !(B.flags[k] & 1u)) return;
   WC_FX_BATCH_ARGS(sA, B, k)
-  fx_acc_body<LEVEL>(sA, bid);
+  fx_acc_body<LEVEL, kFxAccForm>(sA, bid);
+}
+template <int LEVEL, int FORM>
+__global__ void __launch_bounds__(kFxThreads) k_fx_acc_form_b(FxBatch B) {
+  uint32_t bid;
+  const int k = fx_batch_find(B, blockIdx.x, bid);
+  if (LEVEL == 2 && !(B.flags[k] & 1u)) return;
+  WC_FX_BATCH_ARGS(sA, B, k)
+  fx_acc_body<LEVEL, FORM>(sA, bid);
+}
+constexpr uint64_t kFxAccResident = 2000000ull;
+inline int fx_acc_form_of(const wc_ctx *ctx, int level, uint64_t n, uint32_t fmt) {
+  static_assert(kFxAccForm == 3, "fx_launch_acc / fx_launch_acc_b: the cases they name are the NON-default forms");
+  int f = ctx->dev.fx_acc_form & 3;
+  if (ctx->dev.fx_acc_form < 0) f = (n > kFxAccResident && fmt != 2u) ? 1 : kFxAccForm;
+  return level == 2 ? ((f & 2) ? kFxAccForm : 0) : f;
+}
+template <int LEVEL>
+void fx_launch_acc(const wc_ctx *ctx, unsigned grid, hipStream_t st, const FxArgs &A) {
+  const int f = fx_acc_form_of(ctx, LEVEL, A.pts.n, A.fmt);
+  if (f == 0) return (void)k_fx_acc_form<LEVEL, 0><<<grid, kFxThreads, 0, st>>>(A);
+  if constexpr (LEVEL == 1) {
+    if (f == 1) return (void)k_fx_acc_form<1, 1><<<grid, kFxThreads, 0, st>>>(A);
+    if (f == 2) return (void)k_fx_acc_form<1, 2><<<grid, kFxThreads, 0, st>>>(A);
+  }
+  k_fx_acc<LEVEL><<<grid, kFxThreads, 0, st>>>(A);
+}
+template <int LEVEL>
+void fx_launch_acc_b(const wc_ctx *ctx, unsigned grid, hipStream_t st, const FxBatch &B) {
+  const int f = fx_acc_form_of(ctx, LEVEL, 0, 0u);
+  if (f == 0) return (void)k_fx_acc_form_b<LEVEL, 0><<<grid, kFxThreads, 0, st>>>(B);
+  if constexpr (LEVEL == 1) {
+    if (f == 1) return (void)k_fx_acc_form_b<1, 1><<<grid, kFxThreads, 0, st>>>(B);
+    if (f == 2) return (void)k_fx_acc_form_b<1, 2><<<grid, kFxThreads, 0, st>>>(B);
+  }
+  k_fx_acc_b<LEVEL><<<grid, kFxThreads, 0, st>>>(B);
 }
 
 template <int LEVEL>
```
